# microsoft/T-MAC

Measured on AMD Instinct MI355X. Metric: W2A8 GEMV GB/s (llama-2-7B all-layer decode, N=1), higher is better.
Workload: dtype int8

## Files before the change

include/tmac_hip.h:

```cpp
#ifndef TMAC_HIP_H_
#define TMAC_HIP_H_

#include <stddef.h>
#include <stdint.h>

#ifdef __cplusplus
extern "C" {
#endif
#pragma GCC visibility push(default)

#define TMAC_HIP_OK 0
#define TMAC_HIP_E_NOMATCH (-1)
#define TMAC_HIP_E_NODEVICE (-2)
#define TMAC_HIP_E_RUNTIME (-3)
#define TMAC_HIP_E_ARG (-4)

typedef enum { TMAC_F32 = 0, TMAC_F16 = 1 } tmac_dtype_t;

#define TMAC_HIP_ABI_VERSION 1

typedef struct tmac_kcfg {
    int bm;
    int simd_n_in;
    int simd_n_out;
    int kfactor;
    int group_size;
    int lut_scales_size;
    int scales_size;
    int n_tile_num;
    int act_group_size;
    int zero_point;
    int m_groups;
} tmac_kcfg;

typedef struct tmac_hip_weights tmac_hip_weights;
typedef struct tmac_hip_workspace tmac_hip_workspace;

int32_t tmac_hip_init(int device);
const char* tmac_hip_last_error(void);
const char* tmac_hip_version(void);
int32_t tmac_hip_device_count(void);
int32_t tmac_hip_pointer_on_device(const void* p);

int32_t tmac_hip_load_kcfg(const char* path);
int32_t tmac_hip_load_kcfg_ex(const char* path, int replace);
int32_t tmac_hip_clear_kcfg(void);
int32_t tmac_hip_reset_state(void);
int32_t tmac_hip_get_kcfg(int M, int K, int N, int bits, tmac_kcfg* out);
int32_t tmac_hip_set_kcfg(int M, int K, int N, int bits, const tmac_kcfg* cfg);



int32_t tmac_hip_register_weights(tmac_hip_weights** out, const void* A_ref, const void* scales_ref,
                                  int Mw, int K, int bits, const tmac_kcfg* cfg,
                                  tmac_dtype_t host_float, tmac_dtype_t dev_float, void* stream);
int32_t tmac_hip_register_weights_dev(tmac_hip_weights** out, const void* A_ref_dev, const void* scales_ref_dev,
                                      int Mw, int K, int bits, const tmac_kcfg* cfg,
                                      tmac_dtype_t host_float, tmac_dtype_t dev_float, void* stream);
int32_t tmac_hip_free_weights(tmac_hip_weights* w);
size_t tmac_hip_weights_bytes(const tmac_hip_weights* w);

int32_t tmac_hip_workspace_create(tmac_hip_workspace** out, int maxK, int maxN);
int32_t tmac_hip_workspace_free(tmac_hip_workspace* ws);

int32_t tmac_hip_preprocessor_dev(tmac_hip_workspace* ws, const void* B_dev, tmac_dtype_t act_dtype,
                                  int K, int N, int act_group_size, void* stream);

int32_t tmac_hip_qgemm_dev(const tmac_hip_weights* w, const tmac_hip_workspace* ws, void* C_dev,
                           tmac_dtype_t out_dtype, int N, void* stream);

int32_t tmac_hip_qgemm_fused_dev(const tmac_hip_weights* const* weights, int nmat, const void* B_dev,
                                 tmac_dtype_t act_dtype, void* const* C_dev, tmac_dtype_t out_dtype, int N,
                                 void* stream);

int32_t tmac_hip_defer(int on);
int32_t tmac_hip_flush(void* stream);
int32_t tmac_hip_defer_stats(uint64_t* flushes, uint64_t* cache_hits, uint64_t* stream_launches, uint64_t* single_calls);

typedef struct tmac_hip_chain tmac_hip_chain;
int32_t tmac_hip_chain_begin(void);
int32_t tmac_hip_chain_end(tmac_hip_chain** out);
int32_t tmac_hip_chain_abort(void);
int32_t tmac_hip_chain_launch(tmac_hip_chain* chain, void* stream);
int32_t tmac_hip_chain_status(tmac_hip_chain* chain, uint32_t* error_word);
int32_t tmac_hip_chain_info(const tmac_hip_chain* chain, int op, int32_t* nops, int32_t* wpq, int32_t* grid, size_t* bytes);
int32_t tmac_hip_chain_free(tmac_hip_chain* chain);
#define TMAC_XF_NONE 0
#define TMAC_XF_NORM 1
#define TMAC_XF_GLU 2
#define TMAC_XF_GLU_NORM 4
#define TMAC_XF_GATE_SILU  0x000
#define TMAC_XF_GATE_RELU2 0x100
#define TMAC_XF_GATE_GELU  0x200
#define TMAC_XF_CARRY ((const float*)1)
typedef struct {
    int32_t kind;
    const void* in2;
    const float* residual;
    const float* gamma;
    float eps;
    float* residual_out;
    int32_t keep;
} tmac_hip_xform;
int32_t tmac_hip_chain_xform(const tmac_hip_xform* xf);
int32_t tmac_hip_qgemm_fused_xf_dev(const tmac_hip_weights* const* weights, int nmat, const void* B_dev, tmac_dtype_t act_dtype,
                                    const tmac_hip_xform* xf, void* const* C_dev, tmac_dtype_t out_dtype, void* stream);
int32_t tmac_hip_qgemm_fused_xf_rows_dev(const tmac_hip_weights* const* weights, int nmat, const void* B_dev, tmac_dtype_t act_dtype,
                                         const tmac_hip_xform* xf, void* const* C_dev, tmac_dtype_t out_dtype, int N, void* stream);
int32_t tmac_hip_debug_xf_rows_plan(const tmac_hip_weights* const* weights, int nmat, void* const* C_dev, int N, int32_t* route, int32_t* lut);
int32_t tmac_hip_debug_fused_plan(const tmac_hip_weights* const* weights, int nmat, void* const* C_dev, int N, int32_t* route, int32_t* lut);
int32_t tmac_hip_debug_route_stats(uint64_t counts[8]);
int32_t tmac_hip_debug_xf_rows(const void* B_dev, tmac_dtype_t act_dtype, const tmac_hip_xform* xf, int K, int N, float* x_out_dev,
                               void* stream);
#define TMAC_HIP_CHAIN_BLOB_BYTES 128
int32_t tmac_hip_chain_record_gather(const void* send_dev, void* recv_dev, size_t bytes_per_rank, int rank, int world);
int32_t tmac_hip_chain_export(const tmac_hip_chain* chain, void* blob_out);
int32_t tmac_hip_chain_connect(tmac_hip_chain* chain, const void* blobs_of_all_ranks, int world);
int32_t tmac_hip_chain_threads(void);
int32_t tmac_hip_chain_is_stream(const tmac_hip_chain* chain);
int32_t tmac_hip_chain_set_stamps(tmac_hip_chain* chain, unsigned long long* dev_buffer);
int32_t tmac_hip_chain_set_tap(tmac_hip_chain* chain, int32_t* dev_buffer);
int32_t tmac_hip_chain_tap_layout(const tmac_hip_chain* chain, int op, size_t* offset_ints, size_t* count_ints);
int32_t tmac_hip_debug_chain_config(int force_waves_per_quad, unsigned spin_limit);
int32_t tmac_hip_debug_chain_grid(int workgroups);
int32_t tmac_hip_debug_stream_schedule(const double* items, int n, int grid, int ncls, int target, int lpt, int32_t* out_lo, int32_t* out_w, double* out_load);

#define TMAC_HIP_COMM_ID_BYTES 128
typedef struct tmac_hip_comm tmac_hip_comm;
int32_t tmac_hip_comm_unique_id(void* id_out);
int32_t tmac_hip_comm_init(tmac_hip_comm** out, const void* id, int rank, int world);
int32_t tmac_hip_comm_allgather(tmac_hip_comm* comm, const void* send_dev, void* recv_dev, size_t bytes_per_rank, void* stream);
int32_t tmac_hip_comm_destroy(tmac_hip_comm* comm);
#define TMAC_HIP_COMM_BLOB_BYTES 128
int32_t tmac_hip_comm_init_ipc(tmac_hip_comm** out, size_t max_bytes_per_rank, int rank, int world);
int32_t tmac_hip_comm_export(const tmac_hip_comm* comm, void* blob_out);
int32_t tmac_hip_comm_connect(tmac_hip_comm* comm, const void* blobs_of_all_ranks, int world);
int32_t tmac_hip_comm_status(tmac_hip_comm* comm, uint32_t* error_word);
const char* tmac_hip_comm_last_error(void);

int32_t tmac_hip_workspace_ptrs(tmac_hip_workspace* ws, void** qlut_dev, size_t* nbytes_qlut_per_row,
                                void** lut_scales, void** lut_biases);

int32_t tmac_hip_workspace_read(tmac_hip_workspace* ws, int8_t* qlut_host, float* lut_scales_host,
                                float* lut_biases_host, int K, int N, int act_group_size, void* stream);
int32_t tmac_hip_workspace_write(tmac_hip_workspace* ws, const int8_t* qlut_host, const float* lut_scales_host,
                                 const float* lut_biases_host, int K, int N, int act_group_size, void* stream);
int32_t tmac_hip_qgemm_partial_sums(const tmac_hip_weights* w, const tmac_hip_workspace* ws,
                                    int32_t* PS_host, int N, void* stream);
int32_t tmac_hip_qgemm_fused_partial_sums(const tmac_hip_weights* w, const void* B_dev, tmac_dtype_t act_dtype,
                                          int32_t* PS_host, float* C_host, float* lut_host, int N, void* stream);
int32_t tmac_hip_selftest(const uint32_t* in_host, uint32_t* out_host, int n);
int32_t tmac_hip_selftest_mfma(const uint32_t* in_host, int32_t* out_host);
int32_t tmac_hip_set_variant(int variant);
int32_t tmac_hip_set_gemm_min_n(int n);
int32_t tmac_hip_set_fast_aggregation(int mode);
int32_t tmac_hip_debug_stream_read(const void* dev_src, size_t bytes, void* dev_sink, void* stream);
int32_t tmac_hip_debug_quad_config(int force_threads, int force_waves_per_quad);
int32_t tmac_hip_debug_stamps(unsigned long long* dev_buffer);
int32_t tmac_hip_debug_pairs_min_n(int n);
int32_t tmac_hip_debug_gemm_kernel(int which);
int32_t tmac_hip_debug_gemm_stamps(unsigned long long* dev_buffer);
int32_t tmac_hip_debug_gemm_comb_sums(const tmac_hip_weights* w, const tmac_hip_workspace* ws, int32_t* comb_host, int N, void* stream);
int32_t tmac_hip_debug_gemm_image_read(const tmac_hip_workspace* ws, int8_t* half_tables_host, float* lut_scales_host,
                                       float* lut_biases_host, float* entry_sums_host, int N, void* stream);
int32_t tmac_hip_debug_rows_kernel(int mode);
int32_t tmac_hip_debug_rows_stats(uint64_t* launches);
int32_t tmac_hip_debug_rows_plan(int K, int m_groups, int N, int32_t* r_fit, int32_t* ngroups, int32_t* cap, int32_t* live, size_t* lds_bytes);
int32_t tmac_hip_debug_rows_comb_sums(const tmac_hip_weights* w, const tmac_hip_workspace* ws, int32_t* comb_host, int N, void* stream);
int32_t tmac_hip_debug_host_runs(int on);
int32_t tmac_hip_debug_ws_fill_sync(int on);
int32_t tmac_hip_debug_defer_fail(int nth);
int32_t tmac_hip_autotune_fused(const tmac_hip_weights* const* weights, int nmat, tmac_dtype_t act_dtype,
                                tmac_dtype_t out_dtype, int* best_ft, int* best_wpq, float* best_us, float* heuristic_us);
int32_t tmac_hip_tune_save(const char* path);
int32_t tmac_hip_tune_load(const char* path);
int32_t tmac_hip_tune_clear(void);

int32_t qgemm_lut_int8(int m, int k, int n, int b, void* A, void* LUT, void* Scales, void* LUT_Scales,
                       void* LUT_Biases, void* C);
int32_t preprocessor_int8(int m, int k, int n, int b, void* B, void* LUT_Scales, void* LUT_Biases, void* QLUT);
int32_t tmac_hip_cache_clear(void);

#define TMAC_DECL_Q(bm, k, n, b) \
    int32_t qgemm_lut_t1_int8_m##bm##_k##k##_n##n##_b##b(void* A, void* LUT, void* Scales, void* LUT_Scales, void* LUT_Biases, void* C);
#define TMAC_DECL_P(m, k, n, b) \
    int32_t preprocessor_t1_int8_m##m##_k##k##_n##n##_b##b(void* B, void* LUT_Scales, void* LUT_Biases, void* QLUT);
TMAC_DECL_Q(128, 4096, 1, 2) TMAC_DECL_Q(128, 11008, 1, 2)
TMAC_DECL_P(8192, 4096, 1, 2) TMAC_DECL_P(22016, 4096, 1, 2) TMAC_DECL_P(8192, 11008, 1, 2)
TMAC_DECL_Q(1024, 4096, 1, 4) TMAC_DECL_Q(256, 4096, 1, 4) TMAC_DECL_Q(256, 11008, 1, 4)
TMAC_DECL_P(16384, 4096, 1, 4) TMAC_DECL_P(44032, 4096, 1, 4) TMAC_DECL_P(16384, 11008, 1, 4)
TMAC_DECL_Q(256, 4096, 1, 2) TMAC_DECL_Q(512, 4096, 1, 2) TMAC_DECL_Q(128, 14336, 1, 2)
TMAC_DECL_P(28672, 4096, 1, 2) TMAC_DECL_P(8192, 14336, 1, 2) TMAC_DECL_P(2048, 4096, 1, 2)
TMAC_DECL_Q(128, 8640, 1, 2) TMAC_DECL_Q(128, 3200, 1, 2) TMAC_DECL_Q(320, 3200, 1, 2)
TMAC_DECL_P(6400, 8640, 1, 2) TMAC_DECL_P(17280, 3200, 1, 2) TMAC_DECL_P(6400, 3200, 1, 2)
#undef TMAC_DECL_Q
#undef TMAC_DECL_P

#pragma GCC visibility pop
#ifdef __cplusplus
}
#endif
#endif
```

tmac_amd/binding.py:

```python
from __future__ import annotations

import ctypes as C
import os
import subprocess

HERE = os.path.dirname(os.path.abspath(__file__))
F32, F16 = 0, 1
XF_NONE, XF_NORM, XF_GLU, XF_GLU_NORM = 0, 1, 2, 4
XF_GATE_SILU, XF_GATE_RELU2, XF_GATE_GELU = 0x000, 0x100, 0x200


class TMACHipError(RuntimeError):
    def __init__(self, code: int, msg: str):
        super().__init__(f"tmac_hip error {code}: {msg}")
        self.code = code


class XForm(C.Structure):
    _fields_ = [("kind", C.c_int32), ("in2", C.c_void_p), ("residual", C.c_void_p), ("gamma", C.c_void_p), ("eps", C.c_float),
                ("residual_out", C.c_void_p), ("keep", C.c_int32)]


class KCfg(C.Structure):
    _fields_ = [(n, C.c_int) for n in ("bm", "simd_n_in", "simd_n_out", "kfactor", "group_size", "lut_scales_size",
                                       "scales_size", "n_tile_num", "act_group_size", "zero_point", "m_groups")]

    @classmethod
    def make(cls, Mw, K, bits, bm, kfactor=16, group_size=128, act_group_size=64, zero_point=True, m_groups=-1, N=1):
        per = 2 if zero_point else 1
        scales_size = m_groups if m_groups >= 1 else Mw * (K // group_size) * per
        return cls(bm, 16, 8, kfactor, group_size, N * K // act_group_size, scales_size, Mw * bits // bm,
                   act_group_size, int(bool(zero_point)) if m_groups < 1 else 0, m_groups)


def lib_path() -> str:
    return os.environ.get("TMAC_HIP_LIB") or os.path.join(HERE, "lib", "libtmac_hip.so")


def build_library(force: bool = False) -> str:
    if force:
        subprocess.run(["make", "-C", os.path.join(HERE, "csrc"), "clean"], check=True)
    subprocess.run(["make", "-s", "-j4", "-C", os.path.join(HERE, "csrc")], check=True)
    return lib_path()


_lib = None


def load_library() -> C.CDLL:
    global _lib
    if _lib is not None:
        return _lib
    p = lib_path()
    if not os.path.exists(p):
        raise ImportError(f"{p} is missing: build it with `python -c 'import __graft_entry__ as g; g.build()'` "
                          "(hipcc --offload-arch=gfx950); tmac_amd has no fallback path")
    L = C.CDLL(p)
    vp, i32, sz = C.c_void_p, C.c_int32, C.c_size_t
    sigs = {
        "tmac_hip_init": ([C.c_int], i32),
        "tmac_hip_last_error": ([], C.c_char_p),
        "tmac_hip_version": ([], C.c_char_p),
        "tmac_hip_device_count": ([], i32),
        "tmac_hip_pointer_on_device": ([vp], i32),
        "tmac_hip_load_kcfg": ([C.c_char_p], i32),
        "tmac_hip_load_kcfg_ex": ([C.c_char_p, C.c_int], i32),
        "tmac_hip_clear_kcfg": ([], i32),
        "tmac_hip_reset_state": ([], i32),
        "tmac_hip_debug_ws_fill_sync": ([C.c_int], i32),
        "tmac_hip_debug_host_runs": ([C.c_int], i32),
        "tmac_hip_get_kcfg": ([C.c_int] * 4 + [C.POINTER(KCfg)], i32),
        "tmac_hip_set_kcfg": ([C.c_int] * 4 + [C.POINTER(KCfg)], i32),
        "tmac_hip_register_weights": ([C.POINTER(vp), vp, vp, C.c_int, C.c_int, C.c_int, C.POINTER(KCfg), C.c_int, C.c_int, vp], i32),
        "tmac_hip_register_weights_dev": ([C.POINTER(vp), vp, vp, C.c_int, C.c_int, C.c_int, C.POINTER(KCfg), C.c_int, C.c_int, vp], i32),
        "tmac_hip_free_weights": ([vp], i32),
        "tmac_hip_weights_bytes": ([vp], sz),
        "tmac_hip_workspace_create": ([C.POINTER(vp), C.c_int, C.c_int], i32),
        "tmac_hip_workspace_free": ([vp], i32),
        "tmac_hip_preprocessor_dev": ([vp, vp, C.c_int, C.c_int, C.c_int, C.c_int, vp], i32),
        "tmac_hip_qgemm_dev": ([vp, vp, vp, C.c_int, C.c_int, vp], i32),
        "tmac_hip_qgemm_fused_dev": ([C.POINTER(vp), C.c_int, vp, C.c_int, C.POINTER(vp), C.c_int, C.c_int, vp], i32),
        "tmac_hip_qgemm_fused_xf_dev": ([C.POINTER(vp), C.c_int, vp, C.c_int, C.POINTER(XForm), C.POINTER(vp), C.c_int, vp], i32),
        "tmac_hip_qgemm_fused_xf_rows_dev": ([C.POINTER(vp), C.c_int, vp, C.c_int, C.POINTER(XForm), C.POINTER(vp), C.c_int, C.c_int, vp], i32),
        "tmac_hip_debug_xf_rows_plan": ([C.POINTER(vp), C.c_int, C.POINTER(vp), C.c_int, C.POINTER(C.c_int32), C.POINTER(C.c_int32)], i32),
        "tmac_hip_debug_fused_plan": ([C.POINTER(vp), C.c_int, C.POINTER(vp), C.c_int, C.POINTER(C.c_int32), C.POINTER(C.c_int32)], i32),
        "tmac_hip_debug_route_stats": ([C.POINTER(C.c_uint64)], i32),
        "tmac_hip_debug_xf_rows": ([vp, C.c_int, C.POINTER(XForm), C.c_int, C.c_int, vp, vp], i32),
        "tmac_hip_qgemm_fused_partial_sums": ([vp, vp, C.c_int, vp, vp, vp, C.c_int, vp], i32),
        "tmac_hip_workspace_ptrs": ([vp, C.POINTER(vp), C.POINTER(sz), C.POINTER(vp), C.POINTER(vp)], i32),
        "tmac_hip_workspace_read": ([vp, vp, vp, vp, C.c_int, C.c_int, C.c_int, vp], i32),
        "tmac_hip_workspace_write": ([vp, vp, vp, vp, C.c_int, C.c_int, C.c_int, vp], i32),
        "tmac_hip_qgemm_partial_sums": ([vp, vp, vp, C.c_int, vp], i32),
        "tmac_hip_debug_gemm_kernel": ([C.c_int], i32),
        "tmac_hip_debug_gemm_stamps": ([vp], i32),
        "tmac_hip_debug_gemm_comb_sums": ([vp, vp, vp, C.c_int, vp], i32),
        "tmac_hip_debug_rows_kernel": ([C.c_int], i32),
        "tmac_hip_debug_rows_stats": ([C.POINTER(C.c_uint64)], i32),
        "tmac_hip_debug_rows_plan": ([C.c_int, C.c_int, C.c_int, C.POINTER(C.c_int32), C.POINTER(C.c_int32), C.POINTER(C.c_int32), C.POINTER(C.c_int32), C.POINTER(C.c_size_t)], i32),
        "tmac_hip_debug_rows_comb_sums": ([vp, vp, vp, C.c_int, vp], i32),
        "tmac_hip_debug_gemm_image_read": ([vp, vp, vp, vp, vp, C.c_int, vp], i32),
        "tmac_hip_set_variant": ([C.c_int], i32),
        "tmac_hip_set_gemm_min_n": ([C.c_int], i32),
        "tmac_hip_set_fast_aggregation": ([C.c_int], i32),
        "tmac_hip_debug_stream_read": ([vp, sz, vp, vp], i32),
        "tmac_hip_autotune_fused": ([C.c_void_p, C.c_int, C.c_int, C.c_int, C.POINTER(C.c_int), C.POINTER(C.c_int),
                                     C.POINTER(C.c_float), C.POINTER(C.c_float)], i32),
        "tmac_hip_tune_save": ([C.c_char_p], i32),
        "tmac_hip_tune_load": ([C.c_char_p], i32),
        "tmac_hip_tune_clear": ([], i32),
        "tmac_hip_comm_unique_id": ([vp], i32),
        "tmac_hip_comm_init": ([C.POINTER(vp), vp, C.c_int, C.c_int], i32),
        "tmac_hip_comm_allgather": ([vp, vp, vp, sz, vp], i32),
        "tmac_hip_comm_destroy": ([vp], i32),
        "tmac_hip_comm_init_ipc": ([C.POINTER(vp), sz, C.c_int, C.c_int], i32),
        "tmac_hip_comm_export": ([vp, vp], i32),
        "tmac_hip_comm_connect": ([vp, vp, C.c_int], i32),
        "tmac_hip_comm_status": ([vp, C.POINTER(C.c_uint32)], i32),
        "tmac_hip_comm_last_error": ([], C.c_char_p),
        "tmac_hip_defer": ([C.c_int], i32),
        "tmac_hip_flush": ([vp], i32),
        "tmac_hip_debug_defer_fail": ([C.c_int], i32),
        "tmac_hip_defer_stats": ([C.POINTER(C.c_uint64)] * 4, i32),
        "tmac_hip_chain_begin": ([], i32),
        "tmac_hip_chain_end": ([C.POINTER(vp)], i32),
        "tmac_hip_chain_launch": ([vp, vp], i32),
        "tmac_hip_chain_status": ([vp, C.POINTER(C.c_uint32)], i32),
        "tmac_hip_chain_info": ([vp, C.c_int, C.POINTER(i32), C.POINTER(i32), C.POINTER(i32), C.POINTER(sz)], i32),
        "tmac_hip_chain_xform": ([C.POINTER(XForm)], i32),
        "tmac_hip_chain_free": ([vp], i32),
        "tmac_hip_chain_set_stamps": ([vp, vp], i32),
        "tmac_hip_chain_set_tap": ([vp, vp], i32),
        "tmac_hip_chain_tap_layout": ([vp, C.c_int, C.POINTER(sz), C.POINTER(sz)], i32),
        "tmac_hip_chain_threads": ([], i32),
        "tmac_hip_chain_is_stream": ([vp], i32),
        "tmac_hip_chain_record_gather": ([vp, vp, sz, C.c_int, C.c_int], i32),
        "tmac_hip_chain_export": ([vp, vp], i32),
        "tmac_hip_chain_connect": ([vp, vp, C.c_int], i32),
        "tmac_hip_debug_chain_grid": ([C.c_int], i32),
        "tmac_hip_debug_stream_schedule": ([C.POINTER(C.c_double), C.c_int, C.c_int, C.c_int, C.c_int, C.c_int, C.POINTER(C.c_int32), C.POINTER(C.c_int32), C.POINTER(C.c_double)], i32),
        "tmac_hip_debug_chain_config": ([C.c_int, C.c_uint], i32),
        "tmac_hip_debug_quad_config": ([C.c_int, C.c_int], i32),
        "tmac_hip_selftest": ([vp, vp, C.c_int], i32),
        "tmac_hip_selftest_mfma": ([vp, vp], i32),
        "tmac_hip_cache_clear": ([], i32),
        "qgemm_lut_int8": ([C.c_int] * 4 + [vp] * 6, i32),
        "preprocessor_int8": ([C.c_int] * 4 + [vp] * 4, i32),
    }
    optional = {"tmac_hip_chain_is_stream", "tmac_hip_chain_xform", "tmac_hip_qgemm_fused_xf_dev", "tmac_hip_qgemm_fused_xf_rows_dev", "tmac_hip_debug_xf_rows", "tmac_hip_debug_xf_rows_plan", "tmac_hip_debug_fused_plan", "tmac_hip_debug_route_stats", "tmac_hip_comm_init_ipc", "tmac_hip_comm_export", "tmac_hip_comm_connect", "tmac_hip_comm_status",
                "tmac_hip_debug_rows_kernel", "tmac_hip_debug_rows_stats", "tmac_hip_debug_rows_plan", "tmac_hip_debug_rows_comb_sums"} if os.environ.get("TMAC_HIP_LIB") else set()
    for name, (argt, rest) in sigs.items():
        try:
            fn = getattr(L, name)
        except AttributeError:
            if name in optional:
                continue
            raise
        fn.argtypes, fn.restype = argt, rest
    _lib = L
    return L


def lib() -> C.CDLL:
    return load_library()


def check(rc: int) -> None:
    if rc != 0:
        raise TMACHipError(rc, load_library().tmac_hip_last_error().decode())


def check_count(rc: int) -> int:
    if rc < 0:
        raise TMACHipError(rc, load_library().tmac_hip_last_error().decode())
    return rc
```

tmac_amd/csrc/tmac_chain.h:

```cpp
#pragma once
#include <hip/hip_runtime.h>
#include <stdint.h>

namespace tmac {

#ifndef TMAC_CHAIN_FT
#define TMAC_CHAIN_FT 768
#endif
constexpr int CHAIN_FT = TMAC_CHAIN_FT;
constexpr int CHAIN_NWV = CHAIN_FT / 64;
constexpr int CHAIN_RED = 4;
constexpr int CHAIN_US_FLOATS = 48;
constexpr int CHAIN_US_MAX_GROUPS = 8;

struct ChainMat {
    const uint4* W;
    const void* SC;
    void* C;
    uint4* GR;
    int Mw;
    int q_end;
};

struct ChainOp {
    ChainMat m[4];
    int q_end[4];
    const void* in;
    int in_gran;
    int nmat;
    int K, nu, nst, tstride, G, GP, nsg, gs_shift;
    int wpq, ipi;
    int wpq_inv;
    int total_q;
    int q_per, q_extra;
    int m_groups;
    int ipi_inv;
    const void* in2;
    const float* res;
    const float* gamma;
    float* res_out;
    int xf_kind;
    int xf_flags;
    int eps_bits;
    int epi;
    const void* img;
    int img_u4;
    int wg_lo;
};
static_assert(sizeof(ChainOp) == 320, "ChainOp is copied to LDS in 16-byte pieces");

struct ChainArgs {
    const ChainOp* ops;
    int nops;
    unsigned* ctl;
    int out_f16;
    unsigned spin_limit;
    int buf_u4;
    int poll_sleep;
    int poll_delay;
    int issue_first;
    int poll_mode;
    int poll_grid;
    unsigned long long arena_base;
    unsigned long long arena_half;
    unsigned long long peer_base[7];
    int npeer;
    int xforms;
    int carry_floats;
    int tmp_floats, gam_floats;
    int ext_floats;
    int32_t* tap;
    const unsigned long long* tap_off;
    unsigned long long* stamps;
    int gates;
};

hipError_t launch_decode_chain_b1(const ChainArgs& a, bool zp, bool sc_f16, int sm, int grid, size_t lds_bytes, hipStream_t st, int* resident);
hipError_t launch_decode_chain_b2(const ChainArgs& a, bool zp, bool sc_f16, int sm, int grid, size_t lds_bytes, hipStream_t st, int* resident);
hipError_t launch_decode_chain_b3(const ChainArgs& a, bool zp, bool sc_f16, int sm, int grid, size_t lds_bytes, hipStream_t st, int* resident);
hipError_t launch_decode_chain_b4(const ChainArgs& a, bool zp, bool sc_f16, int sm, int grid, size_t lds_bytes, hipStream_t st, int* resident);
hipError_t launch_decode_chain_g2_b1(const ChainArgs& a, bool zp, bool sc_f16, int sm, int grid, size_t lds_bytes, hipStream_t st, int* resident);
hipError_t launch_decode_chain_g2_b2(const ChainArgs& a, bool zp, bool sc_f16, int sm, int grid, size_t lds_bytes, hipStream_t st, int* resident);
hipError_t launch_decode_chain_g2_b3(const ChainArgs& a, bool zp, bool sc_f16, int sm, int grid, size_t lds_bytes, hipStream_t st, int* resident);
hipError_t launch_decode_chain_g2_b4(const ChainArgs& a, bool zp, bool sc_f16, int sm, int grid, size_t lds_bytes, hipStream_t st, int* resident);
inline hipError_t launch_decode_chain(const ChainArgs& a, int bits, bool zp, bool sc_f16, int sm, bool g2, int grid, size_t lds_bytes, hipStream_t st,
                                      int* resident = nullptr) {
    if (g2) {
        switch (bits) {
            case 1: return launch_decode_chain_g2_b1(a, zp, sc_f16, sm, grid, lds_bytes, st, resident);
            case 2: return launch_decode_chain_g2_b2(a, zp, sc_f16, sm, grid, lds_bytes, st, resident);
            case 3: return launch_decode_chain_g2_b3(a, zp, sc_f16, sm, grid, lds_bytes, st, resident);
            case 4: return launch_decode_chain_g2_b4(a, zp, sc_f16, sm, grid, lds_bytes, st, resident);
            default: return hipErrorInvalidValue;
        }
    }
    switch (bits) {
        case 1: return launch_decode_chain_b1(a, zp, sc_f16, sm, grid, lds_bytes, st, resident);
        case 2: return launch_decode_chain_b2(a, zp, sc_f16, sm, grid, lds_bytes, st, resident);
        case 3: return launch_decode_chain_b3(a, zp, sc_f16, sm, grid, lds_bytes, st, resident);
        case 4: return launch_decode_chain_b4(a, zp, sc_f16, sm, grid, lds_bytes, st, resident);
        default: return hipErrorInvalidValue;
    }
}
inline int chain_buf_u4(int K) {
    const int nu = K / 32, nst = (nu + 63) / 64;
    return 4 * 65 * nst + (2 * nst * 32 * 4 + 15) / 16 + CHAIN_US_FLOATS / 4;
}
inline int chain_xf_region_floats(int K) {
    const int P = K / 8, nr = (P + CHAIN_FT - 1) / CHAIN_FT, PS = ((P < CHAIN_FT ? P : CHAIN_FT) + 63) & ~63;
    return nr * 2 * PS * 4;
}
inline size_t chain_lds_bytes(int buf_u4, int nops, int xf_floats = 0) {
    return (size_t)2 * buf_u4 * 16 + sizeof(float) * 2 * CHAIN_NWV * 4 * CHAIN_RED + sizeof(ChainOp) * (size_t)nops + sizeof(float) * (32 + (size_t)xf_floats);
}

#ifndef TMAC_CHAIN_STAMPS
#define TMAC_CHAIN_STAMPS 0
#endif

#ifndef TMAC_STREAM_NLW
#define TMAC_STREAM_NLW 12
#endif
constexpr int STREAM_NLW = TMAC_STREAM_NLW;
constexpr int STREAM_FT = (STREAM_NLW + 1) * 64;
struct StreamArgs {
    const ChainOp* ops;
    int nops;
    int out_f16;
    int buf_u4;
    int nsplit;
    int ncls;
    int vmax;
    const int* nvis;
    const int* roles;
    int32_t* tap;
    const unsigned long long* tap_off;
    unsigned long long* stamps;
};
enum { SR_NST = 0, SR_IPI, SR_NSG, SR_GSH, SR_NU, SR_QE0, SR_QE1, SR_QE2, SR_QPER, SR_QEXTRA, SR_IT_LO, SR_IT_HI, SR_TSTRIDE, SR_OP , SR_WPQ,
       SR_WLO , SR_COMMON };
enum { SRW_NQ = 0 , SRW_NSTEPS, SRW_H, SRW_QS, SRW_INTS };
constexpr int STREAM_ROLE_INTS = SR_COMMON + SRW_INTS * STREAM_NLW;
inline int stream_img_u4(int K) { return (chain_buf_u4(K) + 63) & ~63; }
inline size_t stream_lds_bytes(int buf_u4, int nops, bool qw = false) {
    size_t b = (size_t)2 * buf_u4 * 16 + sizeof(float) * 2 * STREAM_NLW * (qw ? 16 : 4) * CHAIN_RED + sizeof(ChainOp) * (size_t)nops;
#ifdef TMAC_STREAM_STAMPS
    b += 32 * (STREAM_NLW + 1);
#endif
    return b;
}
hipError_t launch_lut_images(const ChainOp* d_ops, int nops, int max_nst, int sm, bool sc_f16, hipStream_t st);
hipError_t launch_gemv_stream(const StreamArgs& a, int bits, bool zp, bool sc_f16, int sm, bool qw, bool g2, int grid, size_t lds_bytes, hipStream_t st);

}
```

tmac_amd/csrc/tmac_chain_host.cpp:

```cpp
#include "tmac_chain_host.h"
#include <algorithm>
#include <array>
#include <memory>
#include <optional>

using namespace tmac_host;

static thread_local std::vector<ChainRecOp>* g_chain_rec = nullptr;
static thread_local std::vector<ChainRecGather>* g_chain_gat = nullptr;
static thread_local std::optional<XfSpec> g_chain_xf;
bool tmac_host::chain_recording() { return g_chain_rec != nullptr; }
void tmac_host::chain_clear_xform() { g_chain_xf.reset(); }

int32_t tmac_host::chain_record(const tmac_hip_weights* const* wl, int nmat, const void* B_dev, tmac_dtype_t act_dtype,
                            void* const* C_list, tmac_dtype_t out_dtype, int N) {
    if (N != 1) { chain_clear_xform(); return fail(TMAC_HIP_E_NOMATCH, "a decode chain records N = 1 calls only"); }
    ChainRecOp op;
    for (int i = 0; i < nmat; ++i) {
        if (!wl[i] || !C_list[i]) { chain_clear_xform(); return fail(TMAC_HIP_E_ARG, "null matrix or output"); }
        op.w.push_back(wl[i]);
        op.C.push_back(C_list[i]);
    }
    op.B = B_dev; op.act = act_dtype; op.out = out_dtype;
    op.xf = g_chain_xf.value_or(XfSpec{});
    chain_clear_xform();
    g_chain_rec->push_back(op);
    return TMAC_HIP_OK;
}

extern "C" int32_t tmac_hip_chain_xform(const tmac_hip_xform* xf) {
    if (!g_chain_rec) return fail(TMAC_HIP_E_ARG, "no chain is being recorded on this thread");
    if (!xf) return fail(TMAC_HIP_E_ARG, "null transform");
    XfSpec spec;
    const int32_t rc = xf_resolve(xf, XF_SITE_CHAIN, &spec);
    if (rc) return rc;
    g_chain_xf = spec;
    return TMAC_HIP_OK;
}

extern "C" int32_t tmac_hip_chain_begin(void) {
    if (g_chain_rec) return fail(TMAC_HIP_E_ARG, "a chain is already being recorded on this thread");
    g_chain_rec = new std::vector<ChainRecOp>();
    g_chain_gat = new std::vector<ChainRecGather>();
    chain_clear_xform();
    return TMAC_HIP_OK;
}

extern "C" int32_t tmac_hip_chain_abort(void) {
    if (!g_chain_rec) return TMAC_HIP_OK;
    delete g_chain_rec;
    delete g_chain_gat;
    g_chain_rec = nullptr;
    g_chain_gat = nullptr;
    chain_clear_xform();
    return TMAC_HIP_OK;
}

extern "C" int32_t tmac_hip_chain_end(tmac_hip_chain** out) {
    if (!g_chain_rec) return fail(TMAC_HIP_E_ARG, "no chain is being recorded on this thread");
    std::vector<ChainRecOp> rec;
    std::vector<ChainRecGather> gat;
    rec.swap(*g_chain_rec);
    gat.swap(*g_chain_gat);
    delete g_chain_rec;
    delete g_chain_gat;
    g_chain_rec = nullptr;
    g_chain_gat = nullptr;
    if (!out) return fail(TMAC_HIP_E_ARG, "null argument");
    return chain_build(rec, gat, out);
}

extern "C" int32_t tmac_hip_chain_record_gather(const void* send_dev, void* recv_dev, size_t bytes_per_rank, int rank, int world) {
    if (!g_chain_rec) return fail(TMAC_HIP_E_ARG, "no chain is being recorded on this thread");
    if (!send_dev || !recv_dev || !bytes_per_rank || world < 1 || world > 8 || rank < 0 || rank >= world)
        return fail(TMAC_HIP_E_ARG, "bad gather (1..8 ranks)");
    g_chain_gat->push_back(ChainRecGather{send_dev, recv_dev, bytes_per_rank, rank, world, g_chain_rec->size()});
    return TMAC_HIP_OK;
}
bool tmac_host::chain_record_gather_if_recording(const void* send_dev, void* recv_dev, size_t bytes_per_rank, int rank, int world, int32_t* rc) {
    if (!g_chain_rec) return false;
    *rc = tmac_hip_chain_record_gather(send_dev, recv_dev, bytes_per_rank, rank, world);
    return true;
}

static int chain_pick_wpq(int total_q, int nst, int grid, int nwv = CHAIN_NWV) {
    int best = 1;
    long best_cost = 1L << 60;
    for (int wpq = 1; wpq <= 4; ++wpq) {
        if (nwv % wpq || (wpq > 1 && wpq > nst)) continue;
        const long ipi = nwv / wpq;
        const long cnt = (total_q + grid - 1) / grid;
        const long iters = (cnt + ipi - 1) / ipi;
        const long steps = (nst + wpq - 1) / wpq;
        if (iters * steps < best_cost) { best_cost = iters * steps; best = wpq; }
    }
    return best;
}

extern "C" int32_t tmac_hip_chain_free(tmac_hip_chain* c) {
    if (!c) return TMAC_HIP_OK;
    const int32_t brc = defer_barrier();
    for (void* p : c->peers) if (p) (void)hipIpcCloseMemHandle(p);
    if (c->arena) (void)hipFree(c->arena);
    if (c->images) (void)hipFree(c->images);
    if (c->d_tap_off) (void)hipFree(c->d_tap_off);
    if (c->d_ops) (void)hipFree(c->d_ops);
    if (c->ctl) (void)hipFree(c->ctl);
    delete c;
    return brc;
}

static void set_wpq(ChainOp& o, int wpq, int nwv) {
    o.wpq = wpq;
    o.ipi = nwv / wpq;
    o.wpq_inv = (65536 + wpq - 1) / wpq;
    o.ipi_inv = (65536 + o.ipi - 1) / o.ipi;
}

static int cls_lo(int cl, int grid, int ncls) { return (cl * grid + ncls - 1) / ncls; }
static void stream_schedule(const std::vector<double>& items, int grid, int ncls, int target, bool lpt, std::vector<int>& blk_lo, std::vector<int>& blk_w,
                            std::vector<std::vector<int>>& visits) {
    const int nop = (int)items.size();
    const double visit_fixed = 8.0;
    blk_lo.assign(nop, 0); blk_w.assign(nop, ncls);
    visits.assign(ncls, std::vector<int>());
    double best_span = 0;
    int best_cap = 0;
    for (int pass = 0; pass < 2; ++pass) {
        for (int cap = ncls; cap >= 1; cap >>= 1) {
            if (pass == 1 && cap != best_cap) continue;
            std::vector<double> load(ncls, 0.0);
            std::vector<std::vector<int>> vis(ncls);
            std::vector<int> order(nop), wof(nop);
            for (int i = 0; i < nop; ++i) {
                int n = 1;
                while (n < cap && items[i] * n / grid < target) n <<= 1;
                order[i] = i; wof[i] = ncls / n;
            }
            if (lpt)
                std::stable_sort(order.begin(), order.end(), [&](int x, int y) {
                    if (wof[x] != wof[y]) return wof[x] > wof[y];
                    return items[x] > items[y];
                });
            for (int oi = 0; oi < nop; ++oi) {
                const int i = order[oi], w = wof[i];
                int bb = 0;
                double bl = 1e300;
                for (int b0 = 0; b0 + w <= ncls; b0 += w) {
                    double m = 0;
                    for (int k = b0; k < b0 + w; ++k) m = load[k] > m ? load[k] : m;
                    if (m < bl) { bl = m; bb = b0; }
                }
                const int wg = cls_lo(bb + w, grid, ncls) - cls_lo(bb, grid, ncls);
                for (int k = bb; k < bb + w; ++k) { load[k] += visit_fixed + items[i] / wg; vis[k].push_back(i); }
                if (pass == 1) { blk_lo[i] = bb; blk_w[i] = w; }
            }
            double span = 0;
            for (int k = 0; k < ncls; ++k) span = load[k] > span ? load[k] : span;
            if (pass == 0 && (best_cap == 0 || span < best_span * 0.999)) { best_span = span; best_cap = cap; }
            if (pass == 1) visits.swap(vis);
        }
    }
}
extern "C" int32_t tmac_hip_debug_stream_schedule(const double* items, int n, int grid, int ncls, int target, int lpt, int32_t* out_lo, int32_t* out_w, double* out_load) {
    if (!items || n < 1 || grid < 1 || ncls < 1 || ncls > 16 || (ncls & (ncls - 1)) || ncls > grid || !out_lo || !out_w) return fail(TMAC_HIP_E_ARG, "bad schedule query");
    std::vector<double> it(items, items + n);
    std::vector<int> lo, w;
    std::vector<std::vector<int>> vis;
    stream_schedule(it, grid, ncls, target, lpt != 0, lo, w, vis);
    for (int i = 0; i < n; ++i) { out_lo[i] = lo[i]; out_w[i] = w[i]; }
    if (out_load)
        for (int k = 0; k < ncls; ++k) {
            out_load[k] = 0;
            for (int i : vis[k]) {
                const int wg = cls_lo(lo[i] + w[i], grid, ncls) - cls_lo(lo[i], grid, ncls);
                out_load[k] += it[i] / wg;
            }
        }
    return TMAC_HIP_OK;
}

static int env_int(const char* name, int dflt) {
    const char* e = getenv(name);
    return e ? atoi(e) : dflt;
}
struct BuildKnobs {
    int wpq = g_knobs.chain_wpq;
    bool glu_epilogue = env_int("TMAC_CHAIN_GLU_EPILOGUE", 1) != 0;
    bool stream = env_int("TMAC_CHAIN_STREAM", 1) != 0;
    int ncls = env_int("TMAC_STREAM_NCLS", 16);
    int visit_items = env_int("TMAC_STREAM_VISIT_ITEMS", 160);
    int qw = env_int("TMAC_STREAM_QW", -1);
    bool lpt = env_int("TMAC_STREAM_LPT", 1) != 0;
    int split = env_int("TMAC_STREAM_SPLIT", 2);
    int split_bits = env_int("TMAC_STREAM_SPLIT_BITS", 3);
    bool split_bits_set = getenv("TMAC_STREAM_SPLIT_BITS") != nullptr;
    int poll_sleep = env_int("TMAC_CHAIN_POLL_SLEEP", 8), poll_delay = env_int("TMAC_CHAIN_POLL_DELAY", 4);
    int issue_first = env_int("TMAC_CHAIN_ISSUE_FIRST", -1), poll_mode = env_int("TMAC_CHAIN_POLL_MODE", 0), poll_grid = env_int("TMAC_CHAIN_POLL_GRID", 0);
    explicit BuildKnobs(int grid) {
        ncls = std::min(std::max(ncls, 1), 16);
        while (ncls > grid || (ncls & (ncls - 1))) --ncls;
    }
};

struct Src { int op, mat; };
struct ChainFlow {
    std::vector<Range> in_r;
    std::vector<std::vector<Range>> out_r;
    std::vector<Src> src, src2;
    std::vector<std::vector<char>> consumed, gathered;
    std::vector<std::vector<char>> dep;
    std::vector<char> epi_of, glu_in_producer;
};
static Src latest_output(const std::vector<ChainRecOp>& rec, const ChainFlow& f, size_t i, const Range& r, const void* p, bool* partial) {
    *partial = false;
    for (size_t j = i; j-- > 0;)
        for (size_t m = 0; m < rec[j].C.size(); ++m)
            if (overlap(r, f.out_r[j][m])) { *partial = rec[j].C[m] != p; return Src{(int)j, (int)m}; }
    return Src{-1, -1};
}
static int32_t analyse_flow(const std::vector<ChainRecOp>& rec, const std::vector<ChainRecGather>& gat, tmac_dtype_t out, ChainFlow& f) {
    const size_t n = rec.size(), out_esz = out == TMAC_F16 ? 2 : 4;
    f.in_r.resize(n); f.out_r.resize(n);
    for (size_t i = 0; i < n; ++i) {
        f.in_r[i] = act_range(rec[i]);
        for (size_t m = 0; m < rec[i].w.size(); ++m) f.out_r[i].push_back(out_range(rec[i], m, out));
        for (size_t m = 0; m < f.out_r[i].size(); ++m)
            for (size_t m2 = 0; m2 < m; ++m2)
                if (overlap(f.out_r[i][m], f.out_r[i][m2])) return fail(TMAC_HIP_E_ARG, "op %zu: outputs %zu and %zu overlap", i, m2, m);
    }
    f.src.assign(n, Src{-1, -1}); f.src2.assign(n, Src{-1, -1});
    f.consumed.resize(n); f.gathered.resize(n);
    for (size_t i = 0; i < n; ++i) { f.consumed[i].assign(rec[i].w.size(), 0); f.gathered[i].assign(rec[i].w.size(), 0); }
    bool partial;
    for (size_t i = 0; i < n; ++i) {
        const ChainRecGather* via = nullptr;
        for (const ChainRecGather& g : gat)
            if (g.pos <= i && g.recv == rec[i].B && (!via || g.pos >= via->pos)) via = &g;
        if (via) {
            for (size_t j = via->pos; j-- > 0 && f.src[i].op < 0;)
                for (size_t m = 0; m < rec[j].C.size(); ++m)
                    if (rec[j].C[m] == via->send) {
                        if (via->bytes != (size_t)rec[j].w[m]->s.Mw * out_esz)
                            return fail(TMAC_HIP_E_ARG, "op %zu: the exchange step gathers %zu bytes per rank, output %zu of op %zu has %zu", i, via->bytes, m, j,
                                        (size_t)rec[j].w[m]->s.Mw * out_esz);
                        if ((size_t)rec[i].w[0]->s.K > (size_t)via->world * rec[j].w[m]->s.Mw)
                            return fail(TMAC_HIP_E_ARG, "op %zu reads %d activations from a gather of %d x %d rows", i, rec[i].w[0]->s.K, via->world, rec[j].w[m]->s.Mw);
                        f.src[i] = Src{(int)j, (int)m};
                        f.consumed[j][m] = 1; f.gathered[j][m] = 1;
                        break;
                    }
            if (f.src[i].op < 0) return fail(TMAC_HIP_E_ARG, "op %zu reads a gathered buffer whose send side no earlier call of the chain writes", i);
            continue;
        }
        const Src s = latest_output(rec, f, i, f.in_r[i], rec[i].B, &partial);
        if (partial)
            return fail(TMAC_HIP_E_NOMATCH, "op %zu reads activations that overlap output %zu of op %zu without being that output: "
                                            "not representable as a hand-off", i, (size_t)s.mat, (size_t)s.op);
        if (s.op >= 0) { f.src[i] = s; f.consumed[s.op][s.mat] = 1; }
    }
    for (size_t i = 0; i < n; ++i) {
        if (!xf_has_glu(rec[i].xf)) continue;
        const Range r2{(const char*)rec[i].xf.in2, (const char*)rec[i].xf.in2 + (size_t)rec[i].w[0]->s.K * 2};
        const Src s = latest_output(rec, f, i, r2, rec[i].xf.in2, &partial);
        if (partial) return fail(TMAC_HIP_E_NOMATCH, "op %zu: the GLU's second vector overlaps output %zu of op %zu without being that output", i, (size_t)s.mat, (size_t)s.op);
        if (s.op >= 0) {
            if (f.gathered[s.op][s.mat]) return fail(TMAC_HIP_E_NOMATCH, "op %zu: a gathered output as the second vector of a GLU is not covered", i);
            f.src2[i] = s; f.consumed[s.op][s.mat] = 1;
        }
        if ((f.src2[i].op >= 0) != (f.src[i].op >= 0))
            return fail(TMAC_HIP_E_NOMATCH, "op %zu: the two vectors of a GLU must both be outputs of the chain or both be external", i);
    }
    f.dep.assign(n, std::vector<char>(n, 0));
    for (size_t k = 0; k < n; ++k) {
        if (f.src[k].op >= 0) {
            f.dep[k] = f.dep[f.src[k].op];
            f.dep[k][f.src[k].op] = 1;
        }
        if (f.src2[k].op >= 0) {
            for (size_t q = 0; q < n; ++q) f.dep[k][q] |= f.dep[f.src2[k].op][q];
            f.dep[k][f.src2[k].op] = 1;
        }
    }
    return TMAC_HIP_OK;
}

static char chain_epi(const XfSpec& s) { return (char)(1 + s.gate); }
static void fill_chain_xf(ChainOp& o, const XfSpec& s, bool in_producer) {
    const bool norm = s.kind == TMAC_XF_NORM, glu_norm = s.kind == TMAC_XF_GLU_NORM;
    o.xf_kind = glu_norm ? TMAC_XF_NORM : (s.kind == TMAC_XF_GLU && in_producer) ? TMAC_XF_NONE : s.kind;
    if (o.xf_kind == TMAC_XF_GLU) o.xf_flags |= s.gate << 8;
    if (norm) {
        o.xf_flags |= (s.carry ? 2 : 0) | (s.keep ? 4 : 0);
        o.res = s.residual; o.res_out = s.residual_out;
    }
    if (norm || glu_norm) { o.gamma = s.gamma; memcpy(&o.eps_bits, &s.eps, 4); }
}

static void plan_glu_epilogue(const std::vector<ChainRecOp>& rec, ChainFlow& f, int grid, const BuildKnobs& kn) {
    const size_t n = rec.size();
    f.epi_of.assign(n, 0); f.glu_in_producer.assign(n, 0);
    if (!kn.glu_epilogue) return;
    std::vector<std::vector<int>> readers(n);
    for (size_t j = 0; j < n; ++j) readers[j].assign(rec[j].w.size(), 0);
    for (size_t i = 0; i < n; ++i) {
        if (f.src[i].op >= 0) ++readers[f.src[i].op][f.src[i].mat];
        if (f.src2[i].op >= 0) ++readers[f.src2[i].op][f.src2[i].mat];
    }
    for (size_t i = 0; i < n; ++i) {
        if (!xf_has_glu(rec[i].xf) || f.src[i].op < 0 || f.src2[i].op != f.src[i].op || f.src[i].mat != 0 || f.src2[i].mat != 1) continue;
        const size_t j = (size_t)f.src[i].op;
        if (rec[j].w.size() != 2 || rec[j].w[0]->s.Mw != rec[j].w[1]->s.Mw || f.gathered[j][0] || f.gathered[j][1] || readers[j][0] != 1 || f.epi_of[j]) continue;
        const Shape& sj = rec[j].w[0]->s;
        const int nqj = 2 * sj.nquads(), nstj = (sj.K / 32 + 63) / 64;
        const int wq = kn.wpq ? kn.wpq : chain_pick_wpq(nqj, nstj, grid);
        if (CHAIN_NWV % wq || ((CHAIN_NWV / wq) & 1)) continue;
        f.epi_of[j] = chain_epi(rec[i].xf); f.glu_in_producer[i] = 1;
        if (readers[j][1] == 1) f.consumed[j][1] = 0;
    }
}

constexpr size_t NO_IMAGE = ~(size_t)0;
struct ChainLayout {
    std::vector<std::array<size_t, 4>> gr;
    std::vector<size_t> in, in2;
    int maxK = 0;
};

static int32_t describe_ops(const std::vector<ChainRecOp>& rec, const ChainFlow& f, const BuildKnobs& kn, tmac_hip_chain& c, ChainLayout& lay) {
    const size_t n = rec.size();
    c.ops.resize(n);
    lay.gr.assign(n, {NO_IMAGE, NO_IMAGE, NO_IMAGE, NO_IMAGE});
    lay.in.assign(n, 0); lay.in2.assign(n, 0);
    for (size_t i = 0; i < n; ++i) {
        const ChainRecOp& r = rec[i];
        ChainOp& o = c.ops[i];
        memset(&o, 0, sizeof(o));
        const Shape& s0 = r.w[0]->s;
        const Src src = f.src[i], src2 = f.src2[i];
        if (r.act != TMAC_F16 && r.act != TMAC_F32) return fail(TMAC_HIP_E_NOMATCH, "op %zu: the decode chain takes fp16 or fp32 activations", i);
        if (r.act == TMAC_F32 && (src.op >= 0 || xf_has_glu(r.xf)))
            return fail(TMAC_HIP_E_NOMATCH, "op %zu: fp32 activations are covered for vectors in memory (an earlier output is handed over as fp16), without a GLU transform", i);
        if ((r.out == TMAC_F16) != (c.out_f16 != 0)) return fail(TMAC_HIP_E_NOMATCH, "op %zu: one output dtype per chain", i);
        if (s0.K > 8 * 3 * CHAIN_FT) return fail(TMAC_HIP_E_NOMATCH, "op %zu: K = %d beyond the decode chain's %d", i, s0.K, 8 * 3 * CHAIN_FT);
        if (((s0.m_groups >= 1) ? 2 : 0) != c.sm) return fail(TMAC_HIP_E_NOMATCH, "op %zu: per-group and unified scales cannot share a chain", i);
        int gu = 1;
        if (c.sm == 2) {
            if (s0.ags != s0.K || s0.K % 64 || s0.m_groups > CHAIN_US_MAX_GROUPS)
                return fail(TMAC_HIP_E_NOMATCH, "op %zu: the unified-scale chain covers one act group per row (act_group_size == K) and up to %d scales per matrix",
                            i, CHAIN_US_MAX_GROUPS);
        } else {
            gu = s0.gs / 32;
            if (s0.ags != 64 || s0.gs < 64 || (gu & (gu - 1)) || s0.K % s0.gs || s0.K % 64)
                return fail(TMAC_HIP_E_NOMATCH, "op %zu: the decode chain covers per-group scales (group >= 64, power of two) with act groups of 64", i);
            if (s0.gs == 64) c.g2 = 1;
        }
        int nq = 0;
        for (size_t m = 0; m < r.w.size(); ++m) {
            const tmac_hip_weights* w = r.w[m];
            const Shape& a = w->s;
            if (layout_of(a) != L_QUAD || !w->tiled_ok || w->fa) return fail(TMAC_HIP_E_NOMATCH, "op %zu matrix %zu is not registered in the QUAD layout", i, m);
            if (a.K != s0.K || a.bits != c.bits || a.gs != s0.gs || a.ags != s0.ags || a.zero_point != c.zp || a.m_groups != s0.m_groups ||
                (w->sc_dtype == F16) != (c.sc_f16 != 0))
                return fail(TMAC_HIP_E_ARG, "op %zu: the matrices of a chain share bits, zero points and scale dtype; those of an op also K and group size", i);
            if (c.sm == 2 && a.Mw % a.m_groups) return fail(TMAC_HIP_E_NOMATCH, "op %zu matrix %zu: rows not divisible by m_groups", i, m);
            nq += a.nquads();
            o.m[m].W = (const uint4*)w->W; o.m[m].SC = w->SC; o.m[m].C = r.C[m]; o.m[m].Mw = a.Mw; o.m[m].q_end = nq;
            if (f.consumed[i][m]) {
                if (r.out != TMAC_F16) return fail(TMAC_HIP_E_NOMATCH, "op %zu: outputs consumed inside the chain must be fp16", i);
                if (f.gathered[i][m] && a.Mw % 4) return fail(TMAC_HIP_E_NOMATCH, "op %zu: row shards of a gathered output must be whole row quads", i);
                const size_t nq_img = (size_t)a.nquads() * (f.gathered[i][m] ? c.world : 1);
                const size_t my_off = f.gathered[i][m] ? (size_t)c.rank * a.nquads() * 16 : 0;
                lay.gr[i][m] = c.arena_bytes + my_off;
                c.layout_hash = (c.layout_hash ^ (nq_img * 16 + i * 4 + m)) * 1099511628211ull;
                c.arena_bytes += (nq_img * 16 + 255) & ~(size_t)255;
            }
            c.bytes += w->w_bytes + w->sc_bytes;
        }
        o.nmat = (int)r.w.size();
        for (int m = 0; m < 4; ++m) o.q_end[m] = (m < o.nmat - 1) ? o.m[m].q_end : 0x7fffffff;
        o.K = s0.K; o.nu = s0.K / 32; o.nst = (o.nu + 63) / 64; o.tstride = o.nst * 64 + 1;
        o.G = s0.K / 64; o.GP = o.nst * 32; o.nsg = c.sm == 2 ? 1 : s0.K / s0.gs;
        o.gs_shift = 0;
        for (int g = gu; g > 1; g >>= 1) ++o.gs_shift;
        o.m_groups = c.sm == 2 ? s0.m_groups : 0;
        o.total_q = nq;
        const int wpq = kn.wpq ? kn.wpq : chain_pick_wpq(nq, o.nst, c.grid);
        if (CHAIN_NWV % wpq) return fail(TMAC_HIP_E_ARG, "waves per quad must divide %d", CHAIN_NWV);
        set_wpq(o, wpq, CHAIN_NWV);
        if (nq / c.grid + 1 + o.ipi >= 4096) return fail(TMAC_HIP_E_NOMATCH, "op %zu: too many rows per workgroup for the decode chain", i);
        o.q_per = nq / c.grid; o.q_extra = nq % c.grid;
        if (f.epi_of[i]) { o.epi = f.epi_of[i]; c.xforms = 1; if (o.epi > 1) c.gates = 1; o.q_per = (nq / 2) / c.grid; o.q_extra = (nq / 2) % c.grid; }
        if (src.op >= 0) {
            const ChainMat& pm = c.ops[src.op].m[src.mat];
            const bool via_gather = f.gathered[src.op][src.mat] != 0;
            if (!via_gather && pm.Mw != o.K) return fail(TMAC_HIP_E_ARG, "op %zu reads an output of %d rows as %d activations", i, pm.Mw, o.K);
            const size_t my_off = via_gather ? (size_t)c.rank * ((pm.Mw + 3) / 4) * 16 : 0;
            lay.in[i] = lay.gr[src.op][src.mat] - my_off; o.in_gran = 1;
        } else {
            o.in = r.B; o.in_gran = 0;
            if (r.act == TMAC_F32) { o.in_gran = 2; c.xforms = 1;
                if (chain_xf_region_floats(s0.K) > c.ext_floats) c.ext_floats = chain_xf_region_floats(s0.K); }
        }
        if (r.xf.kind != TMAC_XF_NONE) {
            const XfSpec& xf = r.xf;
            const int rf = chain_xf_region_floats(o.K);
            const bool reads_glu = xf.kind == TMAC_XF_GLU && !f.glu_in_producer[i];
            const bool runs = xf.kind != TMAC_XF_GLU || reads_glu;
            if (xf.kind == TMAC_XF_GLU_NORM && !f.glu_in_producer[i])
                return fail(TMAC_HIP_E_NOMATCH, "op %zu: a GLU_NORM transform is recorded only where the call in front publishes silu(in) * in2 itself (in and in2 "
                                                "outputs 0 and 1 of one earlier two-matrix call that nothing else reads through a hand-off, not gathered, "
                                                "TMAC_CHAIN_GLU_EPILOGUE != 0, an even number of row quads per workgroup iteration): launch these calls one by one", i);
            if (runs) {
                c.xforms = 1;
                if (o.K > 2 * 8 * CHAIN_FT)
                    return fail(TMAC_HIP_E_NOMATCH, "op %zu: a %s transform is covered up to K = %d%s", i, xf.kind == TMAC_XF_NORM ? "NORM" : xf.kind == TMAC_XF_GLU ? "GLU" : "GLU_NORM",
                                2 * 8 * CHAIN_FT, xf.kind == TMAC_XF_GLU_NORM ? " (the NORM's limit)" : "");
            }
            if (xf.kind == TMAC_XF_NORM) {
                if (o.K > 8192 && (xf.keep || xf.carry)) return fail(TMAC_HIP_E_NOMATCH, "op %zu: a kept residual vector is covered up to K = 8192", i);
                if (xf.carry && c.carry_K != o.K) return fail(TMAC_HIP_E_ARG, "op %zu: no earlier NORM of the chain keeps a vector of %d values", i, o.K);
                if (xf.keep) { c.carry_K = o.K; if (rf > c.carry_floats) c.carry_floats = rf; }
            }
            if (runs && !xf.keep && rf > c.tmp_floats) c.tmp_floats = rf;
            if (xf.gamma && rf > c.gam_floats) c.gam_floats = rf;
            if (reads_glu) {
                if (xf.gate) c.gates = 1;
                if (src2.op >= 0) {
                    const ChainMat& p2 = c.ops[src2.op].m[src2.mat];
                    if (p2.Mw != o.K) return fail(TMAC_HIP_E_ARG, "op %zu: the GLU's second vector has %d rows, K = %d", i, p2.Mw, o.K);
                    lay.in2[i] = lay.gr[src2.op][src2.mat];
                } else o.in2 = xf.in2;
            }
            fill_chain_xf(o, xf, f.glu_in_producer[i] != 0);
        }
        o.in_gran |= 1 << 8;
        if (o.K > lay.maxK) lay.maxK = o.K;
    }
    return TMAC_HIP_OK;
}

static int32_t check_hazards(const std::vector<ChainRecOp>& rec, const ChainFlow& f, const std::vector<ChainOp>& ops) {
    const size_t n = rec.size();
    auto all_past = [&](size_t i, size_t k) {
        for (size_t j = i; j < k; ++j)
            if (f.dep[k][j] && ops[j].q_per >= 1) return true;
        return false;
    };
    for (size_t k = 0; k < n; ++k)
        for (size_t m = 0; m < f.out_r[k].size(); ++m)
            for (size_t i = 0; i < k; ++i) {
                if (f.src[i].op < 0 && overlap(f.out_r[k][m], f.in_r[i]) && !all_past(i, k))
                    return fail(TMAC_HIP_E_NOMATCH, "op %zu overwrites activations that op %zu reads from memory and nothing in the chain orders the two "
                                                    "(no hand-off path from an op in which every workgroup owns rows): launch these calls one by one", k, i);
                for (size_t m2 = 0; m2 < f.out_r[i].size(); ++m2)
                    if (overlap(f.out_r[k][m], f.out_r[i][m2]) && !f.dep[k][i])
                        return fail(TMAC_HIP_E_NOMATCH, "ops %zu and %zu write overlapping outputs and nothing in the chain orders them", i, k);
            }
    std::vector<std::vector<Range>> xf_rd(n);
    std::vector<Range> xf_wr(n, Range{nullptr, nullptr});
    for (size_t i = 0; i < n; ++i) {
        const XfSpec& xf = rec[i].xf;
        const size_t K = (size_t)rec[i].w[0]->s.K;
        if (xf.residual) xf_rd[i].push_back(Range{(const char*)xf.residual, (const char*)xf.residual + K * 4});
        if (xf.in2 && f.src2[i].op < 0) xf_rd[i].push_back(Range{(const char*)xf.in2, (const char*)xf.in2 + K * 2});
        if (xf.gamma) xf_rd[i].push_back(Range{(const char*)xf.gamma, (const char*)xf.gamma + K * 4});
        if (xf.residual_out) xf_wr[i] = Range{(const char*)xf.residual_out, (const char*)xf.residual_out + K * 4};
    }
    for (size_t k = 0; k < n; ++k) {
        for (size_t i = 0; i < n; ++i)
            for (const Range& r : xf_rd[i]) {
                for (size_t m = 0; m < f.out_r[k].size(); ++m)
                    if (overlap(f.out_r[k][m], r) && (i >= k || !all_past(i, k)))
                        return fail(TMAC_HIP_E_NOMATCH, "op %zu writes output %zu over a vector that the transform of op %zu reads from memory and nothing in the "
                                                        "chain orders the writer behind every reader", k, m, i);
                if (xf_wr[k].lo && overlap(xf_wr[k], r) && (i >= k || !all_past(i, k)))
                    return fail(TMAC_HIP_E_NOMATCH, "op %zu: residual_out overlaps a vector that the transform of op %zu reads from memory (a later NORM of the "
                                                    "launch takes the kept vector, TMAC_XF_CARRY)", k, i);
            }
        if (!xf_wr[k].lo) continue;
        for (size_t i = 0; i < n; ++i) {
            if (f.src[i].op < 0 && overlap(xf_wr[k], f.in_r[i]) && (i >= k || !all_past(i, k)))
                return fail(TMAC_HIP_E_NOMATCH, "op %zu: residual_out overlaps activations that op %zu reads from memory", k, i);
            for (size_t m = 0; m < f.out_r[i].size(); ++m)
                if (overlap(xf_wr[k], f.out_r[i][m])) return fail(TMAC_HIP_E_NOMATCH, "op %zu: residual_out overlaps output %zu of op %zu", k, m, i);
            if (i != k && xf_wr[i].lo && overlap(xf_wr[k], xf_wr[i])) return fail(TMAC_HIP_E_NOMATCH, "ops %zu and %zu: overlapping residual_out vectors", i, k);
        }
    }
    return TMAC_HIP_OK;
}

static bool independent(const std::vector<ChainRecOp>& rec, const std::vector<ChainRecGather>& gat, const ChainFlow& f, const std::vector<ChainOp>& ops) {
    if (!gat.empty()) return false;
    for (size_t i = 0; i < rec.size(); ++i)
        if (f.src[i].op >= 0 || f.src2[i].op >= 0 || rec[i].xf.kind != TMAC_XF_NONE || ops[i].epi) return false;
    return true;
}
struct StreamPlan {
    std::vector<ChainOp> ops;
    std::vector<size_t> img_off;
    std::vector<int32_t> roles;
    size_t img_bytes = 0, lds_bytes = 0;
    int buf_u4 = 0, max_nst = 0, ncls = 1, vmax = 1, nsplit = 1;
    bool qw = true;
};
static std::optional<StreamPlan> plan_stream(std::vector<ChainOp> ops, int bits, bool g2, int grid, const BuildKnobs& kn) {
    StreamPlan p;
    p.ops = std::move(ops);
    const int nop = (int)p.ops.size(), ncls = p.ncls = kn.ncls;
    p.img_off.resize(nop);
    for (int i = 0; i < nop; ++i) {
        ChainOp& o = p.ops[i];
        o.img_u4 = stream_img_u4(o.K);
        p.img_off[i] = p.img_bytes;
        p.img_bytes += (size_t)o.img_u4 * 16;
        if (o.img_u4 > p.buf_u4) p.buf_u4 = o.img_u4;
        if (o.nst > p.max_nst) p.max_nst = o.nst;
        o.in_gran &= 2;
    }
    const int nwv = STREAM_NLW;
    {
        double it64 = 0, it16 = 0;
        for (const ChainOp& o : p.ops) {
            for (int m = 0; m < o.nmat; ++m) if (((o.m[m].Mw + 3) / 4) % 4) p.qw = false;
            it64 += (double)o.total_q * o.nst; it16 += (double)(o.total_q / 4) * ((o.nu + 15) / 16);
        }
        if (kn.qw == 0 || (kn.qw < 0 && bits >= 3 && it16 > 0.85 * it64)) p.qw = false;
    }
    const bool qw = p.qw;
    auto op_q = [&](const ChainOp& o) { return qw ? o.total_q / 4 : o.total_q; };
    auto op_nst = [&](const ChainOp& o) { return qw ? (o.nu + 15) / 16 : o.nst; };
    std::vector<int> blk_lo, blk_w;
    std::vector<std::vector<int>> visits;
    {
        std::vector<double> items(nop);
        for (int i = 0; i < nop; ++i) items[i] = (double)op_q(p.ops[i]) * op_nst(p.ops[i]);
        stream_schedule(items, grid, ncls, kn.visit_items, kn.lpt, blk_lo, blk_w, visits);
    }
    for (int i = 0; i < nop; ++i) {
        ChainOp& o = p.ops[i];
        const int wlo = cls_lo(blk_lo[i], grid, ncls), wcnt = cls_lo(blk_lo[i] + blk_w[i], grid, ncls) - wlo;
        o.wg_lo = wlo;
        const int tq = op_q(o), nstw = op_nst(o);
        set_wpq(o, (!kn.wpq || nwv % o.wpq || o.wpq > nstw) ? chain_pick_wpq(tq, nstw, wcnt, nwv) : o.wpq, nwv);
        o.q_per = tq / wcnt; o.q_extra = tq % wcnt;
        if (tq / wcnt + 1 + o.ipi >= 4096) return std::nullopt;
        if (qw) for (int m = 0; m < 4; ++m) { if (o.q_end[m] != 0x7fffffff) o.q_end[m] /= 4; o.m[m].q_end /= 4; }
    }
    int vmax = 1;
    for (int k = 0; k < ncls; ++k) if ((int)visits[k].size() > vmax) vmax = (int)visits[k].size();
    p.vmax = vmax;
    const size_t lds2 = stream_lds_bytes(p.buf_u4, (vmax + 1) / 2, qw);
    p.lds_bytes = stream_lds_bytes(p.buf_u4, vmax, qw);
    const int split_bits = (g2 && !kn.split_bits_set && kn.split_bits > 2) ? 2 : kn.split_bits;
    if (kn.split >= 2 && bits <= split_bits && vmax >= 2 && 2 * lds2 + 2048 <= 160 * 1024) { p.nsplit = 2; p.lds_bytes = lds2; }
    for (int ns = 3; ns <= kn.split && ns <= 4; ++ns) {
        const size_t ldsn = stream_lds_bytes(p.buf_u4, (vmax + ns - 1) / ns, qw);
        if (p.nsplit == ns - 1 && vmax >= ns && ns * (ldsn + 1024) <= 160 * 1024) { p.nsplit = ns; p.lds_bytes = ldsn; }
    }
    if (p.lds_bytes > 160 * 1024) return std::nullopt;
    p.roles.assign((size_t)STREAM_ROLE_INTS * ncls * vmax + ncls, 0);
    for (int k = 0; k < ncls; ++k) {
        p.roles[(size_t)STREAM_ROLE_INTS * ncls * vmax + k] = (int32_t)visits[k].size();
        for (size_t v = 0; v < visits[k].size(); ++v) {
            const int i = visits[k][v];
            const ChainOp& o = p.ops[i];
            int32_t* r = p.roles.data() + ((size_t)k * vmax + v) * STREAM_ROLE_INTS;
            const int nstw = op_nst(o);
            r[SR_NST] = nstw; r[SR_IPI] = o.ipi; r[SR_NSG] = o.nsg; r[SR_GSH] = o.gs_shift; r[SR_NU] = o.nu;
            r[SR_QE0] = o.q_end[0]; r[SR_QE1] = o.q_end[1]; r[SR_QE2] = o.q_end[2];
            r[SR_QPER] = o.q_per; r[SR_QEXTRA] = o.q_extra;
            r[SR_IT_LO] = (o.q_per + o.ipi - 1) / o.ipi; r[SR_IT_HI] = (o.q_per + o.ipi) / o.ipi;
            r[SR_TSTRIDE] = o.tstride; r[SR_OP] = i; r[SR_WPQ] = o.wpq; r[SR_WLO] = o.wg_lo;
            for (int wl = 0; wl < STREAM_NLW; ++wl) {
                int32_t* rw = r + SR_COMMON + SRW_INTS * wl;
                const int qs = wl / o.wpq, h = wl - qs * o.wpq;
                auto nq = [&](int cnt) { return qs < cnt ? (cnt - 1 - qs) / o.ipi + 1 : 0; };
                rw[SRW_NQ] = nq(o.q_per) | (nq(o.q_per + 1) << 16);
                rw[SRW_NSTEPS] = h < nstw ? (nstw - h + o.wpq - 1) / o.wpq : 0;
                rw[SRW_H] = h; rw[SRW_QS] = qs;
            }
        }
    }
    return p;
}

static int32_t commit_stream(tmac_hip_chain& c, StreamPlan& p) {
    const size_t role_bytes = p.roles.size() * sizeof(int32_t);
    if (hipMalloc(&c.images, p.img_bytes + role_bytes) != hipSuccess || hipMemset(c.images, 0, p.img_bytes) != hipSuccess ||
        hipMemcpy(static_cast<char*>(c.images) + p.img_bytes, p.roles.data(), role_bytes, hipMemcpyHostToDevice) != hipSuccess)
        return fail(TMAC_HIP_E_RUNTIME, "LUT image allocation failed (%zu bytes)", p.img_bytes + role_bytes);
    c.roles = reinterpret_cast<const int*>(static_cast<char*>(c.images) + p.img_bytes);
    c.nvis = c.roles + (size_t)STREAM_ROLE_INTS * p.ncls * p.vmax;
    c.ncls = p.ncls; c.vmax = p.vmax; c.qw = p.qw; c.nsplit = p.nsplit; c.max_nst = p.max_nst;
    c.ops = std::move(p.ops);
    for (size_t i = 0; i < c.ops.size(); ++i) c.ops[i].img = static_cast<const char*>(c.images) + p.img_off[i];
    c.stream = true; c.buf_u4 = p.buf_u4; c.lds_bytes = p.lds_bytes; c.xforms = 0;
    return TMAC_HIP_OK;
}
static int32_t commit(tmac_hip_chain& c, const ChainLayout& lay) {
    if (!c.stream) {
        c.buf_u4 = chain_buf_u4(lay.maxK);
        c.lds_bytes = chain_lds_bytes(c.buf_u4, (int)c.ops.size(), c.carry_floats + c.tmp_floats + c.gam_floats + c.ext_floats);
        if (c.lds_bytes > 160 * 1024)
            return fail(TMAC_HIP_E_NOMATCH, "%zu calls with K up to %d need %zu bytes of LDS (LUT buffers + call descriptors): record shorter chains",
                        c.ops.size(), lay.maxK, c.lds_bytes);
        ChainArgs probe;
        memset(&probe, 0, sizeof(probe));
        probe.nops = 1;
        int resident = 0;
        hipError_t e = launch_decode_chain(probe, c.bits, c.zp != 0, c.sc_f16 != 0, c.sm, c.g2 != 0, c.grid, c.lds_bytes, nullptr, &resident);
        if (e == hipErrorInvalidValue) return fail(TMAC_HIP_E_NOMATCH, "no decode-chain kernel for this configuration");
        if (e != hipSuccess || resident < 1)
            return fail(TMAC_HIP_E_NOMATCH, "the decode chain's workgroup does not fit a compute unit (%s, %zu bytes of LDS)",
                        e == hipSuccess ? "occupancy 0" : hipGetErrorString(e), c.lds_bytes);
    }
    if (c.arena_bytes) {
        const hipError_t ea = c.world > 1 ? hipExtMallocWithFlags(&c.arena, 2 * c.arena_bytes, hipDeviceMallocFinegrained)
                                          : hipMalloc(&c.arena, 2 * c.arena_bytes);
        if (ea != hipSuccess || hipMemset(c.arena, 0, 2 * c.arena_bytes) != hipSuccess)
            return fail(TMAC_HIP_E_RUNTIME, "hand-off arena allocation failed (%zu bytes)", 2 * c.arena_bytes);
        char* const base = static_cast<char*>(c.arena);
        for (size_t i = 0; i < c.ops.size(); ++i) {
            ChainOp& o = c.ops[i];
            for (int m = 0; m < o.nmat; ++m)
                if (lay.gr[i][m] != NO_IMAGE) o.m[m].GR = reinterpret_cast<uint4*>(base + lay.gr[i][m]);
            if (o.in_gran & 1) o.in = base + lay.in[i];
            if ((o.in_gran & 1) && o.xf_kind == TMAC_XF_GLU) o.in2 = base + lay.in2[i];
        }
    }
    c.connected = c.world == 1;
    if (hipMalloc((void**)&c.d_ops, sizeof(ChainOp) * c.ops.size()) != hipSuccess ||
        hipMemcpy(c.d_ops, c.ops.data(), sizeof(ChainOp) * c.ops.size(), hipMemcpyHostToDevice) != hipSuccess)
        return fail(TMAC_HIP_E_RUNTIME, "descriptor upload failed");
    const unsigned ctl0[4] = {1u, 0u, 0u, 0u};
    if (hipMalloc((void**)&c.ctl, sizeof(ctl0)) != hipSuccess || hipMemcpy(c.ctl, ctl0, sizeof(ctl0), hipMemcpyHostToDevice) != hipSuccess)
        return fail(TMAC_HIP_E_RUNTIME, "control word allocation failed");
    if (hipStreamSynchronize(nullptr) != hipSuccess) return fail(TMAC_HIP_E_RUNTIME, "hand-off buffer initialisation failed");
    return TMAC_HIP_OK;
}

struct ChainFree { void operator()(tmac_hip_chain* c) const { (void)tmac_hip_chain_free(c); } };

int32_t tmac_host::chain_build(const std::vector<ChainRecOp>& rec, const std::vector<ChainRecGather>& gat, tmac_hip_chain** out) {
    *out = nullptr;
    if (rec.empty()) return fail(TMAC_HIP_E_ARG, "nothing was recorded");
    int32_t rc = ensure_device();
    if (rc) return rc;
    int dev = 0, cus = 0;
    HIP_TRY(hipGetDevice(&dev));
    HIP_TRY(hipDeviceGetAttribute(&cus, hipDeviceAttributeMultiprocessorCount, dev));
    if (cus < 1) return fail(TMAC_HIP_E_RUNTIME, "no compute units reported");
    std::unique_ptr<tmac_hip_chain, ChainFree> c(new tmac_hip_chain());
    c->grid = (g_knobs.chain_grid > 0 && g_knobs.chain_grid < cus) ? g_knobs.chain_grid : cus;
    const BuildKnobs kn(c->grid);
    for (const ChainRecGather& g : gat) {
        if (g.world != gat[0].world || g.rank != gat[0].rank) return fail(TMAC_HIP_E_ARG, "the exchange steps of a chain share rank and world size");
        c->rank = g.rank; c->world = g.world;
    }
    const tmac_hip_weights* w0 = rec[0].w[0];
    c->bits = w0->s.bits; c->zp = w0->s.zero_point; c->sc_f16 = w0->sc_dtype == F16; c->out_f16 = rec[0].out == TMAC_F16;
    c->sm = (w0->s.m_groups >= 1) ? 2 : 0;
    if (c->bits < 1 || c->bits > 4) return fail(TMAC_HIP_E_NOMATCH, "the decode chain is built for 1- to 4-bit weights");

    ChainFlow flow;
    if ((rc = analyse_flow(rec, gat, rec[0].out, flow)) != TMAC_HIP_OK) return rc;
    plan_glu_epilogue(rec, flow, c->grid, kn);
    ChainLayout lay;
    if ((rc = describe_ops(rec, flow, kn, *c, lay)) != TMAC_HIP_OK) return rc;
    if ((rc = check_hazards(rec, flow, c->ops)) != TMAC_HIP_OK) return rc;
    std::optional<StreamPlan> plan;
    if (kn.stream && independent(rec, gat, flow, c->ops)) plan = plan_stream(c->ops, c->bits, c->g2 != 0, c->grid, kn);
    if (plan && (rc = commit_stream(*c, *plan)) != TMAC_HIP_OK) return rc;
    if ((rc = commit(*c, lay)) != TMAC_HIP_OK) return rc;
    c->poll_sleep = kn.poll_sleep; c->poll_delay = kn.poll_delay; c->issue_first = kn.issue_first; c->poll_mode = kn.poll_mode; c->poll_grid = kn.poll_grid;
    *out = c.release();
    return TMAC_HIP_OK;
}

extern "C" int32_t tmac_hip_debug_chain_grid(int workgroups) {
    if (workgroups < 0) return fail(TMAC_HIP_E_ARG, "negative grid");
    g_knobs.chain_grid = workgroups;
    return TMAC_HIP_OK;
}

extern "C" int32_t tmac_hip_debug_chain_config(int force_wpq, unsigned spin_limit) {
    if (force_wpq < 0 || (force_wpq && CHAIN_NWV % force_wpq)) return fail(TMAC_HIP_E_ARG, "waves per quad must divide %d", CHAIN_NWV);
    g_knobs.chain_wpq = force_wpq;
    if (spin_limit) g_knobs.chain_spin_limit = spin_limit;
    return TMAC_HIP_OK;
}
```

tmac_amd/csrc/tmac_chain_host.h:

```cpp
#pragma once
#include "tmac_host.h"

struct tmac_hip_chain {
    std::vector<tmac::ChainOp> ops;
    tmac::ChainOp* d_ops = nullptr;
    unsigned* ctl = nullptr;
    void* arena = nullptr;
    size_t arena_bytes = 0;
    unsigned long long layout_hash = 0;
    int rank = 0, world = 1;
    std::vector<void*> peers;
    bool connected = false;
    int bits = 0, zp = 0, sc_f16 = 0, out_f16 = 0;
    int sm = 0;
    int grid = 0, buf_u4 = 0;
    size_t lds_bytes = 0;
    unsigned long long* stamps = nullptr;
    int32_t* tap = nullptr;
    unsigned long long* d_tap_off = nullptr;
    size_t bytes = 0;
    int xforms = 0, carry_floats = 0;
    int gates = 0;
    int tmp_floats = 0, gam_floats = 0, ext_floats = 0, carry_K = 0;
    int poll_sleep = 8, poll_delay = 4, issue_first = -1, poll_mode = 0, poll_grid = 0;
    hipStream_t last_stream = nullptr;
    bool launched = false;
    bool stream = false;
    void* images = nullptr;
    int max_nst = 0;
    const int* roles = nullptr;
    const int* nvis = nullptr;
    int ncls = 1, vmax = 0;
    bool qw = false;
    int nsplit = 1;
    int g2 = 0;
};

namespace tmac_host {

struct ChainRecOp {
    std::vector<const tmac_hip_weights*> w;
    const void* B;
    std::vector<void*> C;
    tmac_dtype_t act, out;
    XfSpec xf;
};
struct ChainRecGather {
    const void* send;
    const void* recv;
    size_t bytes;
    int rank, world;
    size_t pos;
};

struct Range { const char* lo; const char* hi; };
inline bool overlap(const Range& a, const Range& b) { return a.lo < b.hi && b.lo < a.hi; }
inline Range act_range(const ChainRecOp& r) { return Range{(const char*)r.B, (const char*)r.B + (size_t)r.w[0]->s.K * (r.act == TMAC_F32 ? 4 : 2)}; }
inline Range out_range(const ChainRecOp& r, size_t m, tmac_dtype_t out) {
    return Range{(const char*)r.C[m], (const char*)r.C[m] + (size_t)r.w[m]->s.Mw * (out == TMAC_F16 ? 2 : 4)};
}

int32_t chain_build(const std::vector<ChainRecOp>& rec, const std::vector<ChainRecGather>& gat, tmac_hip_chain** out);

}
```

tmac_amd/csrc/tmac_chain_launch.cpp:

```cpp
#include "tmac_chain_host.h"

using namespace tmac_host;

extern "C" int32_t tmac_hip_chain_launch(tmac_hip_chain* c, void* stream) {
    bind_thread_device();
    const int32_t brc = defer_barrier();
    if (brc) return brc;
    if (!c) return fail(TMAC_HIP_E_ARG, "null chain");
    hipStream_t st = (hipStream_t)stream;
    if (c->launched && st != c->last_stream && hipStreamQuery(c->last_stream) != hipSuccess) {
        (void)hipGetLastError();
        return fail(TMAC_HIP_E_ARG, "the chain is still in flight on another stream: synchronise it first, or record one chain per stream");
    }
    if (!c->connected) return fail(TMAC_HIP_E_ARG, "a row-sharded chain must be connected to its peers first (tmac_hip_chain_export / tmac_hip_chain_connect)");
    if (c->stream) {
        hipError_t e = launch_lut_images(c->d_ops, (int)c->ops.size(), c->max_nst, c->sm, c->sc_f16 != 0, st);
        if (e != hipSuccess) return fail(TMAC_HIP_E_RUNTIME, "LUT image launch: %s", hipGetErrorString(e));
        StreamArgs sa;
        memset(&sa, 0, sizeof(sa));
        sa.ops = c->d_ops; sa.nops = (int)c->ops.size(); sa.out_f16 = c->out_f16; sa.buf_u4 = c->buf_u4; sa.nsplit = c->nsplit; sa.roles = c->roles; sa.stamps = c->stamps;
        sa.ncls = c->ncls; sa.vmax = c->vmax; sa.nvis = c->nvis; sa.tap = c->tap; sa.tap_off = c->d_tap_off;
        e = launch_gemv_stream(sa, c->bits, c->zp != 0, c->sc_f16 != 0, c->sm, c->qw, c->g2 != 0, c->grid, c->lds_bytes, st);
        if (e != hipSuccess) return fail(TMAC_HIP_E_RUNTIME, "stream launch: %s", hipGetErrorString(e));
        c->last_stream = st; c->launched = true;
        return TMAC_HIP_OK;
    }
    ChainArgs a;
    memset(&a, 0, sizeof(a));
    a.ops = c->d_ops; a.nops = (int)c->ops.size(); a.ctl = c->ctl; a.out_f16 = c->out_f16;
    a.arena_base = reinterpret_cast<unsigned long long>(c->arena); a.arena_half = c->arena_bytes;
    a.npeer = (int)c->peers.size();
    for (int p = 0; p < a.npeer; ++p) a.peer_base[p] = reinterpret_cast<unsigned long long>(c->peers[p]);
    a.spin_limit = g_knobs.chain_spin_limit; a.buf_u4 = c->buf_u4; a.stamps = c->stamps;
    a.xforms = c->xforms; a.gates = c->gates; a.carry_floats = c->carry_floats; a.tmp_floats = c->tmp_floats; a.gam_floats = c->gam_floats; a.ext_floats = c->ext_floats;
    {
        static const int force_xf = [] { const char* e = getenv("TMAC_HIP_CHAIN_FORCE_XF"); return e && e[0] == '1' ? 1 : 0; }();
        if (force_xf) a.xforms = 1;
    }
    if (c->tap) { a.tap = c->tap; a.tap_off = c->d_tap_off; a.xforms = 1; }
    a.poll_sleep = c->poll_sleep; a.poll_delay = c->poll_delay; a.issue_first = c->issue_first; a.poll_mode = c->poll_mode; a.poll_grid = c->poll_grid;
    hipError_t e = launch_decode_chain(a, c->bits, c->zp != 0, c->sc_f16 != 0, c->sm, c->g2 != 0, c->grid, c->lds_bytes, st);
    if (e == hipErrorInvalidValue) return fail(TMAC_HIP_E_NOMATCH, "no decode-chain kernel for this configuration");
    if (e != hipSuccess) return fail(TMAC_HIP_E_RUNTIME, "decode chain launch: %s", hipGetErrorString(e));
    c->last_stream = st; c->launched = true;
    return TMAC_HIP_OK;
}

struct ChainBlob {
    hipIpcMemHandle_t handle;
    unsigned long long arena_bytes, layout_hash;
    int rank, world;
};
static_assert(sizeof(ChainBlob) <= TMAC_HIP_CHAIN_BLOB_BYTES, "blob size");

extern "C" int32_t tmac_hip_chain_export(const tmac_hip_chain* c, void* blob_out) {
    if (!c || !blob_out) return fail(TMAC_HIP_E_ARG, "null argument");
    if (!c->arena) return fail(TMAC_HIP_E_ARG, "the chain hands nothing over");
    ChainBlob b;
    memset(&b, 0, sizeof(b));
    HIP_TRY(hipIpcGetMemHandle(&b.handle, c->arena));
    b.arena_bytes = 2 * c->arena_bytes; b.layout_hash = c->layout_hash; b.rank = c->rank; b.world = c->world;
    memset(blob_out, 0, TMAC_HIP_CHAIN_BLOB_BYTES);
    memcpy(blob_out, &b, sizeof(b));
    return TMAC_HIP_OK;
}

extern "C" int32_t tmac_hip_chain_connect(tmac_hip_chain* c, const void* blobs, int world) {
    if (!c || !blobs) return fail(TMAC_HIP_E_ARG, "null argument");
    if (world != c->world) return fail(TMAC_HIP_E_ARG, "the chain was recorded for %d ranks, %d blobs given", c->world, world);
    if (c->connected && c->world > 1) return fail(TMAC_HIP_E_ARG, "the chain is already connected");
    bind_thread_device();
    for (int r = 0; r < world; ++r) {
        ChainBlob b;
        memcpy(&b, (const char*)blobs + (size_t)r * TMAC_HIP_CHAIN_BLOB_BYTES, sizeof(b));
        if (b.rank != r || b.world != world || b.arena_bytes != 2 * c->arena_bytes || b.layout_hash != c->layout_hash)
            return fail(TMAC_HIP_E_ARG, "rank %d recorded a different chain (its blob does not match this rank's hand-off layout)", r);
        if (r == c->rank) continue;
        void* p = nullptr;
        hipError_t e = hipIpcOpenMemHandle(&p, b.handle, hipIpcMemLazyEnablePeerAccess);
        if (e != hipSuccess) {
            for (void* q : c->peers) if (q) (void)hipIpcCloseMemHandle(q);
            c->peers.clear();
            return fail(TMAC_HIP_E_RUNTIME, "hipIpcOpenMemHandle of rank %d's hand-off arena: %s", r, hipGetErrorString(e));
        }
        c->peers.push_back(p);
    }
    c->connected = true;
    return TMAC_HIP_OK;
}

extern "C" int32_t tmac_hip_chain_status(tmac_hip_chain* c, uint32_t* error_word) {
    if (!c || !error_word) return fail(TMAC_HIP_E_ARG, "null argument");
    unsigned ctl[4];
    HIP_TRY(hipMemcpy(ctl, c->ctl, sizeof(ctl), hipMemcpyDeviceToHost));
    *error_word = ctl[2];
    if (ctl[2] || ctl[1]) {
        if (ctl[1] && c->world > 1)
            return fail(TMAC_HIP_E_RUNTIME, "a row-sharded chain was interrupted inside a launch (%u of its workgroups exited): the ranks' generations differ now -- "
                                            "free the chain on every rank, record and connect it again", ctl[1]);
        if (ctl[1] && c->arena) HIP_TRY(hipMemset(c->arena, 0, 2 * c->arena_bytes));
        const unsigned fresh[4] = {ctl[0], 0u, 0u, 0u};
        HIP_TRY(hipMemcpy(c->ctl, fresh, sizeof(fresh), hipMemcpyHostToDevice));
    }
    return TMAC_HIP_OK;
}

extern "C" int32_t tmac_hip_chain_info(const tmac_hip_chain* c, int op, int32_t* nops, int32_t* wpq, int32_t* grid, size_t* bytes) {
    if (!c) return fail(TMAC_HIP_E_ARG, "null chain");
    if (nops) *nops = (int32_t)c->ops.size();
    if (grid) *grid = c->grid;
    if (bytes) *bytes = c->bytes;
    if (wpq) {
        if (op < 0 || op >= (int)c->ops.size()) return fail(TMAC_HIP_E_ARG, "op index out of range");
        *wpq = c->ops[op].wpq;
    }
    return TMAC_HIP_OK;
}

static std::vector<unsigned long long> tap_offsets(const tmac_hip_chain* c) {
    std::vector<unsigned long long> off(c->ops.size() + 1, 0);
    for (size_t i = 0; i < c->ops.size(); ++i)
        off[i + 1] = off[i] + (unsigned long long)4 * c->ops[i].total_q * (c->sm == 2 ? c->bits : c->ops[i].G);
    return off;
}
extern "C" int32_t tmac_hip_chain_tap_layout(const tmac_hip_chain* c, int op, size_t* offset_ints, size_t* count_ints) {
    if (!c) return fail(TMAC_HIP_E_ARG, "null chain");
    if (op < 0 || op > (int)c->ops.size()) return fail(TMAC_HIP_E_ARG, "op index out of range");
    const std::vector<unsigned long long> off = tap_offsets(c);
    if (offset_ints) *offset_ints = (size_t)off[op];
    if (count_ints) *count_ints = op < (int)c->ops.size() ? (size_t)(off[op + 1] - off[op]) : 0;
    return TMAC_HIP_OK;
}
extern "C" int32_t tmac_hip_chain_set_tap(tmac_hip_chain* c, int32_t* dev_buffer) {
    if (!c) return fail(TMAC_HIP_E_ARG, "null chain");
    if (!dev_buffer) { c->tap = nullptr; return TMAC_HIP_OK; }
    for (const ChainOp& o : c->ops)
        if (o.epi) return fail(TMAC_HIP_E_NOMATCH, "the tap does not cover calls whose row quads are dealt in gate / up pairs (GLU in the producer)");
    bind_thread_device();
    if (!c->d_tap_off) {
        const std::vector<unsigned long long> off = tap_offsets(c);
        if (hipMalloc((void**)&c->d_tap_off, off.size() * sizeof(unsigned long long)) != hipSuccess ||
            hipMemcpy(c->d_tap_off, off.data(), off.size() * sizeof(unsigned long long), hipMemcpyHostToDevice) != hipSuccess)
            return fail(TMAC_HIP_E_RUNTIME, "tap offsets: allocation failed");
    }
    c->tap = dev_buffer;
    return TMAC_HIP_OK;
}

extern "C" int32_t tmac_hip_chain_set_stamps(tmac_hip_chain* c, unsigned long long* dev_buffer) {
    if (!c) return fail(TMAC_HIP_E_ARG, "null chain");
#ifndef TMAC_STREAM_STAMPS
    if (c->stream && dev_buffer) return fail(TMAC_HIP_E_NOMATCH, "stamps of a stream-mode chain exist in -DTMAC_STREAM_STAMPS builds only (layout: StreamArgs::stamps)");
#endif
    if (!c->stream && dev_buffer && !TMAC_CHAIN_STAMPS)
        return fail(TMAC_HIP_E_NOMATCH, "stamps of k_decode_chain exist in -DTMAC_CHAIN_STAMPS=1 builds of the library only (tools/build_variant.sh)");
    c->stamps = dev_buffer;
    return TMAC_HIP_OK;
}

extern "C" int32_t tmac_hip_chain_threads(void) { return CHAIN_FT; }

extern "C" int32_t tmac_hip_chain_is_stream(const tmac_hip_chain* c) { return c && c->stream ? (c->qw ? 2 : 1) : 0; }
```

tmac_amd/csrc/tmac_stream.hip:

```cpp
#include <hip/hip_runtime.h>
#include <hip/hip_fp16.h>
#include <stdint.h>

#include "tmac_chain_core.h"

#ifndef TMAC_STREAM_QW_TU
#define TMAC_STREAM_QW_TU 0
#endif
#ifndef TMAC_STREAM_G2_TU
#define TMAC_STREAM_G2_TU 0
#endif

namespace tmac {

#if !TMAC_STREAM_QW_TU && !TMAC_STREAM_G2_TU
__global__ __launch_bounds__(256) void k_lut_images(const ChainOp* __restrict__ ops) {
    const ChainOp& d = ops[blockIdx.y];
    const int K = d.K, P = K / 8, nst = d.nst;
    if ((int)blockIdx.x >= nst) return;
    const int p = blockIdx.x * 256 + threadIdx.x;
    uint4* tab = reinterpret_cast<uint4*>(const_cast<void*>(d.img));
    float* l_sc = reinterpret_cast<float*>(tab + IMG2_STEP * nst);
    uint4* tslot = tab + img2_index(p >> 2, p & 3);
#if TMAC_IMG2_SC
    float* scslot = l_sc + 4 * (p >> 4) + ((p >> 3) & 1);
#else
    float* scslot = l_sc + (p >> 3);
#endif
    if (p >= P) {
        *tslot = make_uint4(0u, 0u, 0u, 0u);
        if ((p & 7) == 0) { scslot[0] = 0.f; scslot[TMAC_IMG2_SC ? 2 : 32 * nst] = 0.f; }
        return;
    }
    float x[8];
    if (d.in_gran & 2) {
        const float4* src = reinterpret_cast<const float4*>(d.in) + 2 * (size_t)p;
        const float4 a0 = src[0], a1 = src[1];
        x[0] = a0.x; x[1] = a0.y; x[2] = a0.z; x[3] = a0.w; x[4] = a1.x; x[5] = a1.y; x[6] = a1.z; x[7] = a1.w;
    } else {
        const uint4 v = reinterpret_cast<const uint4*>(d.in)[p];
        const uint32_t r[4] = {v.x, v.y, v.z, v.w};
#pragma unroll
        for (int i = 0; i < 4; ++i) {
            const __half2 hh = *reinterpret_cast<const __half2*>(&r[i]);
            x[2 * i] = __low2float(hh); x[2 * i + 1] = __high2float(hh);
        }
    }
    const float s0 = __fadd_rn(__fadd_rn(fabsf(x[0]), fabsf(x[1])), __fadd_rn(fabsf(x[2]), fabsf(x[3])));
    const float s1 = __fadd_rn(__fadd_rn(fabsf(x[4]), fabsf(x[5])), __fadd_rn(fabsf(x[6]), fabsf(x[7])));
    const float mx = q_half_allmax(fmaxf(s0, s1));
    const float scales = div127(mx);
    const float t_scales = (scales != 0.0f) ? rcp_exact(scales) : 0.0f;
    uint32_t lo0, hi0, lo1, hi1;
    float La, Lb;
    q_table8<true>(x[0], x[1], x[2], x[3], t_scales, lo0, hi0, La);
    q_table8<true>(x[4], x[5], x[6], x[7], t_scales, lo1, hi1, Lb);
    *tslot = make_uint4(lo0, hi0, lo1, hi1);
    float va = -La, vb = -Lb;
    va = __fadd_rn(va, qdpp_f<0x4E>(va));
    vb = __fadd_rn(vb, qdpp_f<0x4E>(vb));
    va = __fadd_rn(va, qdpp_f<0xB1>(va));
    vb = __fadd_rn(vb, qdpp_f<0xB1>(vb));
    const float v = __fadd_rn(va, vb);
    const float c1 = qdpp_f<0x104>(v);
    if ((p & 7) == 0) {
        scslot[0] = __fmul_rn(0.5f, scales);
        scslot[TMAC_IMG2_SC ? 2 : 32 * nst] = __fmul_rn(0.5f, __fadd_rn(__fadd_rn(0.0f, v), c1));
    }
}

template <bool SCF16>
__global__ __launch_bounds__(256) void k_lut_images_us(const ChainOp* __restrict__ ops) {
    __shared__ float s_cs[768];
    __shared__ float s_mx[4];
    const ChainOp& d = ops[blockIdx.x];
    const int K = d.K, P = K / 8, nu = d.nu, nst = d.nst;
    const int tid = threadIdx.x, w = tid >> 6, lane = tid & 63;
    uint4* tab = reinterpret_cast<uint4*>(const_cast<void*>(d.img));
    float* l_us = reinterpret_cast<float*>(tab + IMG2_STEP * nst);
    auto load8 = [&](int p, float (&x)[8]) __attribute__((always_inline)) {
        if (d.in_gran & 2) {
            const float4* src = reinterpret_cast<const float4*>(d.in) + 2 * (size_t)p;
            const float4 a0 = src[0], a1 = src[1];
            x[0] = a0.x; x[1] = a0.y; x[2] = a0.z; x[3] = a0.w; x[4] = a1.x; x[5] = a1.y; x[6] = a1.z; x[7] = a1.w;
        } else {
            const uint4 v = reinterpret_cast<const uint4*>(d.in)[p];
            const uint32_t r[4] = {v.x, v.y, v.z, v.w};
#pragma unroll
            for (int i = 0; i < 4; ++i) {
                const __half2 hh = *reinterpret_cast<const __half2*>(&r[i]);
                x[2 * i] = __low2float(hh); x[2 * i + 1] = __high2float(hh);
            }
        }
    };
    float mx = 0.f;
    for (int p = tid; p < P; p += 256) {
        float x[8];
        load8(p, x);
        mx = fmaxf(mx, __fadd_rn(__fadd_rn(fabsf(x[0]), fabsf(x[1])), __fadd_rn(fabsf(x[2]), fabsf(x[3]))));
        mx = fmaxf(mx, __fadd_rn(__fadd_rn(fabsf(x[4]), fabsf(x[5])), __fadd_rn(fabsf(x[6]), fabsf(x[7]))));
        float va = -__fadd_rn(__fadd_rn(__fadd_rn(x[0], x[1]), x[2]), x[3]);
        float vb = -__fadd_rn(__fadd_rn(__fadd_rn(x[4], x[5]), x[6]), x[7]);
        va = __fadd_rn(va, qdpp_f<0x4E>(va));
        vb = __fadd_rn(vb, qdpp_f<0x4E>(vb));
        va = __fadd_rn(va, qdpp_f<0xB1>(va));
        vb = __fadd_rn(vb, qdpp_f<0xB1>(vb));
        if ((p & 3) == 0) s_cs[p >> 2] = __fadd_rn(va, vb);
    }
    mx = q_row_allmax(mx);
    mx = q_xor_max_f(mx);
    if (lane == 0) s_mx[w] = mx;
    __syncthreads();
    mx = fmaxf(fmaxf(s_mx[0], s_mx[1]), fmaxf(s_mx[2], s_mx[3]));
    const float gscale = div127(mx);
    const float gtinv = (gscale != 0.0f) ? rcp_exact(gscale) : 0.0f;
    for (int p = tid; p < P; p += 256) {
        float x[8];
        load8(p, x);
        uint32_t lo0, hi0, lo1, hi1;
        float La, Lb;
        q_table8<true>(x[0], x[1], x[2], x[3], gtinv, lo0, hi0, La);
        q_table8<true>(x[4], x[5], x[6], x[7], gtinv, lo1, hi1, Lb);
        tab[img2_index(p >> 2, p & 3)] = make_uint4(lo0, hi0, lo1, hi1);
    }
    for (int j4 = 0; j4 < 4; ++j4)
        for (int u = nu + tid; u < nst * 64; u += 256) tab[img2_index(u, j4)] = make_uint4(0u, 0u, 0u, 0u);
    if (tid == 0) {
        float biases = 0.0f;
        for (int c = 0; c < nu; ++c) biases = __fadd_rn(biases, s_cs[c]);
        l_us[0] = gscale;
        l_us[1] = biases;
    }
    if (tid >= 64 && tid < 64 + 4 * CHAIN_US_MAX_GROUPS) {
        const int mi = (tid - 64) / CHAIN_US_MAX_GROUPS, g = (tid - 64) % CHAIN_US_MAX_GROUPS;
        if (mi < d.nmat && g < d.m_groups)
            l_us[16 + mi * CHAIN_US_MAX_GROUPS + g] = SCF16 ? __half2float(reinterpret_cast<const __half*>(d.m[mi].SC)[g]) : reinterpret_cast<const float*>(d.m[mi].SC)[g];
    }
}

hipError_t launch_lut_images(const ChainOp* d_ops, int nops, int max_nst, int sm, bool sc_f16, hipStream_t st) {
    if (nops < 1 || max_nst < 1) return hipErrorInvalidValue;
    if (sm == 2 && sc_f16) hipLaunchKernelGGL(k_lut_images_us<true>, dim3(nops), dim3(256), 0, st, d_ops);
    else if (sm == 2) hipLaunchKernelGGL(k_lut_images_us<false>, dim3(nops), dim3(256), 0, st, d_ops);
    else hipLaunchKernelGGL(k_lut_images, dim3(max_nst, nops), dim3(256), 0, st, d_ops);
    return hipGetLastError();
}
#endif

#ifndef TMAC_STREAM_KO
#define TMAC_STREAM_KO 0
#endif
#define TMAC_STREAM_ATTR __attribute__((amdgpu_num_sgpr(82)))
template <int BITS, bool ZP, bool SCF16, int RING, int MINW, int SM, bool TAP, bool QW, bool G2 = false>
__global__ __launch_bounds__(STREAM_FT, MINW) TMAC_STREAM_ATTR void k_gemv_stream(StreamArgs a) {
    extern __shared__ __attribute__((aligned(16))) uint4 lds[];
    constexpr int NWV = STREAM_NLW;
    constexpr int RPW = QW ? 16 : 4;
    const int tid = threadIdx.x, w = __builtin_amdgcn_readfirstlane(tid >> 6), lane = tid & 63;
    const int nsplit = a.nsplit, part = (int)blockIdx.x % nsplit, bx = (int)blockIdx.x / nsplit;
    const int cls = __builtin_amdgcn_readfirstlane(bx * a.ncls / ((int)gridDim.x / nsplit));
    const int* my_roles = a.roles + (size_t)cls * a.vmax * STREAM_ROLE_INTS;
    const int nops = max((a.nvis[cls] - part + nsplit - 1) / nsplit, 0);
    if (nops == 0) return;
    float* l_red = reinterpret_cast<float*>(lds + 2 * (size_t)a.buf_u4);
    uint4* l_ops = lds + 2 * (size_t)a.buf_u4 + (2 * NWV * RPW * CHAIN_RED * sizeof(float)) / 16;
    {
        constexpr int U = (int)(sizeof(ChainOp) / 16);
        const uint4* gsrc = reinterpret_cast<const uint4*>(a.ops);
        for (int idx = tid; idx < nops * U; idx += STREAM_FT) {
            const int jl = idx / U, r = idx - jl * U;
            l_ops[idx] = gsrc[my_roles[(size_t)(jl * nsplit + part) * STREAM_ROLE_INTS + SR_OP] * U + r];
        }
        __syncthreads();
    }
    const cop_ptr ops = reinterpret_cast<cop_ptr>(l_ops);
    auto wg_iters = [&](cop_ptr d) __attribute__((always_inline)) {
        const int qper = uni(d->q_per), qex = uni(d->q_extra), ipi = uni(d->ipi), iinv = uni(d->ipi_inv), bl = bx - uni(d->wg_lo);
        const int cnt = qper + (bl < qex ? 1 : 0);
        return ((cnt + ipi - 1) * iinv) >> 16;
    };

    if (w == NWV) {
        typedef __attribute__((address_space(3))) void* lds_vp;
        const uint32_t lds0 = (uint32_t)(uintptr_t)(__attribute__((address_space(3))) uint4*)lds;
        auto load_image = [&](int j) __attribute__((always_inline)) {
            const cop_ptr d = ops + j;
            const int n16 = uni(d->img_u4);
            const __amdgpu_buffer_rsrc_t rs = __builtin_amdgcn_make_buffer_rsrc(const_cast<void*>(uni(d->img)), (short)0, n16 * 16, 0x00020000);
            const uint32_t base = lds0 + (uint32_t)(j & 1) * (uint32_t)a.buf_u4 * 16u;
            for (int o = 0; o < n16; o += 64)
                __builtin_amdgcn_raw_ptr_buffer_load_lds(rs, (lds_vp)(uintptr_t)(base + (uint32_t)o * 16u), 16, (o + lane) * 16, 0, 0, 0);
        };
        int s_par = 0;
        auto combine = [&](int j, int t, int par) __attribute__((always_inline)) {
            const cop_ptr d = ops + j;
            const int qper = uni(d->q_per), qex = uni(d->q_extra), ipi = uni(d->ipi), wpq = uni(d->wpq), bl = bx - uni(d->wg_lo);
            const int q_lo = bl * qper + min(bl, qex), cnt = qper + (bl < qex ? 1 : 0);
            constexpr int SPP = 64 / RPW;
            for (int pass = 0; pass * SPP < ipi; ++pass) {
            const int p_qs = pass * SPP + (int)((unsigned)lane / RPW), p_row = lane & (RPW - 1);
            const int p_gql = q_lo + t * ipi + p_qs;
            if (p_qs < ipi && p_gql < q_lo + cnt) {
                const int e0 = uni(d->q_end[0]), e1 = uni(d->q_end[1]), e2 = uni(d->q_end[2]);
                const int p_mi = (p_gql >= e0 ? 1 : 0) + (p_gql >= e1 ? 1 : 0) + (p_gql >= e2 ? 1 : 0);
                const int p_lq = p_gql - (p_gql >= e2 ? e2 : (p_gql >= e1 ? e1 : (p_gql >= e0 ? e0 : 0)));
                const unsigned long long p_c = reinterpret_cast<unsigned long long>(d->m[p_mi].C);
                const float* red = l_red + par * (NWV * RPW * CHAIN_RED);
                float v;
                if (SM == 2) {
                    int32_t cb[BITS];
#pragma unroll
                    for (int pl = 0; pl < BITS; ++pl) cb[pl] = 0;
                    const int32_t* redi = reinterpret_cast<const int32_t*>(red);
                    for (int ww = 0; ww < wpq; ++ww)
#pragma unroll
                        for (int pl = 0; pl < BITS; ++pl) cb[pl] += redi[((p_qs * wpq + ww) * RPW + p_row) * CHAIN_RED + pl];
                    if constexpr (TAP) {
                        if (a.tap) {
                            const int opi = my_roles[(size_t)(j * nsplit + part) * STREAM_ROLE_INTS + SR_OP];
#pragma unroll
                            for (int pl = 0; pl < BITS; ++pl) a.tap[a.tap_off[opi] + (size_t)(RPW * p_gql + p_row) * BITS + pl] = cb[pl];
                        }
                    }
                    float acc = 0.f;
#pragma unroll
                    for (int pl = 0; pl < BITS; ++pl) {
                        const float tp = __fmul_rn((float)cb[pl], q_alpha(pl));
                        acc = (pl == 0) ? tp : __fadd_rn(acc, tp);
                    }
                    const float* l_us = reinterpret_cast<const float*>(lds + (size_t)(j & 1) * a.buf_u4 + IMG2_STEP * (size_t)uni(d->nst));
                    const float vv = __fadd_rn(__fmul_rn(acc, l_us[0]), __fmul_rn(l_us[1], 0.5f));
                    const int mg = uni(d->m_groups);
                    const int g = mg == 1 ? 0 : (RPW * p_lq + p_row) / (d->m[p_mi].Mw / mg);
                    v = __fmul_rn(vv, l_us[16 + p_mi * CHAIN_US_MAX_GROUPS + g]);
                } else {
                v = red[((p_qs * wpq) * RPW + p_row) * CHAIN_RED];
                for (int ww = 1; ww < wpq; ++ww) v = __fadd_rn(v, red[((p_qs * wpq + ww) * RPW + p_row) * CHAIN_RED]);
                }
                asm volatile("" : "+v"(v));
                const size_t oi = (size_t)(RPW * p_lq + p_row);
                if (a.out_f16) c_store_b16(p_c + 2 * oi, (uint32_t)__half_as_ushort(__float2half_rn(v)));
                else c_store_b32(p_c + 4 * oi, __float_as_uint(v));
            }
            }
        };
        load_image(0);
        int prev_nit = 0;
        for (int j = 0; j < nops; ++j) {
            asm volatile("s_waitcnt vmcnt(0)" ::: "memory");
            c_lds_barrier();
            if (!(TMAC_STREAM_KO & 1) && j > 0 && prev_nit > 0) combine(j - 1, prev_nit - 1, s_par ^ 1);
            if (!(TMAC_STREAM_KO & 4) && j + 1 < nops) load_image(j + 1);
            const int nit = wg_iters(ops + j);
            if (!(TMAC_STREAM_KO & 2))
                for (int t = 0; t < nit; ++t) {
                    c_lds_barrier();
                    if (!(TMAC_STREAM_KO & 1) && t + 1 < nit) combine(j, t, s_par);
                    s_par ^= 1;
                }
            prev_nit = nit;
        }
        if (!(TMAC_STREAM_KO & 1) && prev_nit > 0) combine(nops - 1, prev_nit - 1, s_par ^ 1);
        return;
    }

    CSel<BITS> sel;
    c_selectors<BITS, SM>(sel, lane);
    uint32_t k3 = 0x03020100u;
    asm volatile("" : "+v"(k3));
    uint32_t lane16 = QW ? (uint32_t)(lane & 15) * 16u : (uint32_t)lane * 16u;
    asm volatile("" : "+v"(lane16));
    uint32_t lk4 = QW ? 8u * (uint32_t)(lane >> 4)
                      : 4u * (uint32_t)(2 * (lane & 12) + 2 * (lane >> 4));
    asm volatile("" : "+v"(lk4));
    const int wl = NWV - 1 - w;

    typedef int sr16 __attribute__((ext_vector_type(16)));
    typedef int sr4 __attribute__((ext_vector_type(4)));
    auto load_role = [&](int jl, sr16& rc, sr4& rw) __attribute__((always_inline)) {
        const int* rp = my_roles + (size_t)(jl * nsplit + part) * STREAM_ROLE_INTS;
        const int* rpw = rp + SR_COMMON + SRW_INTS * wl;
        asm volatile("s_load_dwordx16 %0, %2, 0x0\n\ts_load_dwordx4 %1, %3, 0x0\n\ts_waitcnt lgkmcnt(0)" : "=&s"(rc), "=&s"(rw) : "s"(rp), "s"(rpw) : "memory");
    };
    auto items_of = [&](const sr16& rc, const sr4& rw) __attribute__((always_inline)) {
        const int nq = bx - rc[SR_WLO] < rc[SR_QEXTRA] ? (int)((unsigned)rw[SRW_NQ] >> 16) : (rw[SRW_NQ] & 0xffff);
        return nq * rw[SRW_NSTEPS];
    };

    CFrag<BITS, G2> ring[RING];
    const __amdgpu_buffer_rsrc_t null_rs = __builtin_amdgcn_make_buffer_rsrc(static_cast<uint4*>(nullptr), (short)0, 0, 0x00020000);
    const TMAC_GLOBAL char* ops_g = as_global(reinterpret_cast<const char*>(a.ops));
    const uint32_t dummy_boff = (uint32_t)(lane & 3) * (uint32_t)((ZP ? 2 : 1) * (SCF16 ? 2 : 4));
    uint32_t v_sc0 = dummy_boff;
    bool i_rag = false;
    uint32_t v_wq = lane16, v_scq = dummy_boff;
    int i_op = -1, i_left = 0, i_st = 0, i_h = 0, i_wpq = 1, i_nst = 1, i_nsg1 = 0, i_gsh = 0, i_nu = 0, i_gq = 0, i_ipi = 1, i_n64 = 1;
    int q_lo = 0, q_hi = 0, q_woff = 0;
    bool q_stale = true;
    cop_ptr i_d = ops;
    __amdgpu_buffer_rsrc_t q_rs = null_rs;
    const TMAC_GLOBAL char* q_sc = ops_g;
    const TMAC_GLOBAL char* q_scm = ops_g;
    int q_scstride = 0;
    const uint32_t c0 = QW ? (uint32_t)(4 * (lane >> 4)) : (uint32_t)(4 * (lane & 12) + 4 * (lane >> 4));
    uint32_t c0g = c0;
    int i_sc2 = 0;
    constexpr int SC_SHIFT = (ZP ? 1 : 0) + (SCF16 ? 3 : 4);
    auto refill = [&](CFrag<BITS, G2>& f) __attribute__((always_inline)) {
        while (i_left == 0 && i_op < nops) {
            ++i_op;
            if (i_op < nops) {
                i_d = ops + i_op;
                sr16 rc; sr4 rw;
                load_role(i_op, rc, rw);
                i_left = items_of(rc, rw);
                i_st = rw[SRW_H]; i_h = rw[SRW_H]; i_wpq = rc[SR_WPQ]; i_nst = rc[SR_NST]; i_ipi = rc[SR_IPI];
                const int bl = bx - rc[SR_WLO];
                i_gq = bl * rc[SR_QPER] + min(bl, rc[SR_QEXTRA]) + rw[SRW_QS];
                i_nsg1 = rc[SR_NSG] - 1; i_gsh = rc[SR_GSH]; i_nu = rc[SR_NU];
                q_scstride = rc[SR_NSG] << SC_SHIFT;
                c0g = c0 >> i_gsh;
                if constexpr (G2) i_sc2 = i_gsh < 2 ? 1 << SC_SHIFT : 0;
                if constexpr (QW) {
                    i_n64 = (rc[SR_TSTRIDE] - 1) >> 6;
                    v_wq = (uint32_t)(lane >> 4) * (uint32_t)(i_n64 * (BITS * 1024)) + lane16;
                    v_scq = (uint32_t)((lane >> 2) & 3) * (uint32_t)q_scstride + dummy_boff;
                    v_sc0 = (c0g << SC_SHIFT) + v_scq;
                    i_rag = (i_nu & 15) != 0;
                } else {
                    v_sc0 = (c0g << SC_SHIFT) | dummy_boff;
                    i_rag = (i_nu & 63) != 0;
                }
                q_hi = 0; q_stale = true;
            }
        }
        const bool real = i_left > 0;
        if (real && q_stale) {
            if (i_gq >= q_hi) {
                const int e0 = uni(i_d->q_end[0]), e1 = uni(i_d->q_end[1]), e2 = uni(i_d->q_end[2]);
                const int mi = (i_gq >= e0 ? 1 : 0) + (i_gq >= e1 ? 1 : 0) + (i_gq >= e2 ? 1 : 0);
                q_lo = i_gq >= e2 ? e2 : (i_gq >= e1 ? e1 : (i_gq >= e0 ? e0 : 0));
                q_hi = i_gq >= e2 ? 0x7fffffff : (i_gq >= e1 ? e2 : (i_gq >= e0 ? e1 : e0));
                q_rs = __builtin_amdgcn_make_buffer_rsrc(const_cast<uint4*>(uni(i_d->m[mi].W)), (short)0, 0x7fffffff, 0x00020000);
                q_scm = as_global(uni(reinterpret_cast<const char*>(i_d->m[mi].SC)));
            }
            const int lq = QW ? 4 * (i_gq - q_lo) : i_gq - q_lo;
            q_sc = q_scm + (size_t)lq * (size_t)q_scstride;
            q_woff = lq * (QW ? i_n64 : i_nst) * (BITS * 1024);
            q_stale = false;
        }
        CItemOps io;
        if (real) {
            io.rs = q_rs;
            const int ub = QW ? i_st << 4 : i_st << 6;
            if (i_rag && i_st == i_nst - 1) {
                const uint32_t sg = min((uint32_t)(ub >> i_gsh) + c0g, (uint32_t)i_nsg1);
                io.sc = q_sc;
                io.boff = QW ? (sg << SC_SHIFT) + v_scq : ((sg << SC_SHIFT) | dummy_boff);
                if constexpr (G2) {
                    const uint32_t sg2 = min((uint32_t)(ub >> i_gsh) + c0g + (uint32_t)(i_sc2 >> SC_SHIFT), (uint32_t)i_nsg1);
                    io.boff2 = QW ? (sg2 << SC_SHIFT) + v_scq : ((sg2 << SC_SHIFT) | dummy_boff);
                }
                io.l16 = QW ? v_wq : ((lane < i_nu - ub) ? lane16 : 0u);
            } else {
                io.sc = q_sc + ((size_t)(ub >> i_gsh) << SC_SHIFT);
                io.boff = v_sc0;
                if constexpr (G2) io.boff2 = v_sc0 + (uint32_t)i_sc2;
                io.l16 = QW ? v_wq : lane16;
            }
            io.soff = QW ? q_woff + (i_st >> 2) * (BITS * 1024) + (i_st & 3) * 256 : q_woff + i_st * (BITS * 1024);
        } else { io.rs = null_rs; io.soff = 0; io.sc = ops_g; io.boff = dummy_boff; io.l16 = 0u; if constexpr (G2) io.boff2 = dummy_boff; }
        c_issue_static<BITS, ZP, SCF16, SM, G2>(f, io);
        if (real) {
            --i_left;
            i_st += i_wpq;
            if (i_st >= i_nst) { i_st = i_h; i_gq += i_ipi; q_stale = true; }
        }
    };
#pragma unroll
    for (int k = 0; k < RING; ++k) refill(ring[k]);

    int c_op = -1, c_left = 0, c_it = 0, c_st = 0, parity = 0, my_iter = 0;
    int tstride = 1, nst = 1, wpq = 1, h = 0;
    int t_gq0 = 0, t_ipi = 1, t_G = 0;
    int32_t* t_base = nullptr;
    uint4* tab = lds;
    float* l_ls = reinterpret_cast<float*>(lds);
    float* l_lb = l_ls;
    float cacc = 0.f;
    int32_t iacc[BITS];
#pragma unroll
    for (int pl = 0; pl < BITS; ++pl) iacc[pl] = 0;

#ifdef TMAC_STREAM_STAMPS
    uint32_t* t_lds = reinterpret_cast<uint32_t*>(l_ops) + (size_t)nops * (sizeof(ChainOp) / 4) + (size_t)w * 8;
    if (lane < 8) t_lds[lane] = 0;
    uint32_t t_prev = (uint32_t)__builtin_readcyclecounter();
#if TMAC_STREAM_STAMPS >= 2
    if (lane == 0) t_lds[7] = 0u - t_prev;
#else
    if (lane == 0) { t_lds[6] = t_prev; t_lds[7] = (uint32_t)(__builtin_readcyclecounter() >> 32); }
#endif
#if TMAC_STREAM_STAMPS >= 2
#define TMAC_ST(i) do { const uint32_t t_now = (uint32_t)__builtin_readcyclecounter(); if (lane == 0) (void)__hip_atomic_fetch_add(&t_lds[i], t_now - t_prev, __ATOMIC_RELAXED, __HIP_MEMORY_SCOPE_WORKGROUP); t_prev = t_now; } while (0)
#else
#define TMAC_ST(i) do { } while (0)
#endif
#else
#define TMAC_ST(i) do { } while (0)
#endif
    auto finish = [&](bool have, float acc_in) __attribute__((always_inline)) {
        if (TMAC_STREAM_KO & 2) { ++c_it; return; }
        float* red = l_red + parity * (NWV * RPW * CHAIN_RED);
        if (SM == 2) {
            int32_t* redi = reinterpret_cast<int32_t*>(red);
#pragma unroll
            for (int pl = 0; pl < BITS; ++pl) {
                uint32_t v = have ? (uint32_t)iacc[pl] : 0u;
                if constexpr (!QW) {
                    v += qdpp_u<0x124>(v);
                    v += qdpp_u<0x128>(v);
                }
                v = q_xor_add_u(v);
                if (lane < RPW) redi[(wl * RPW + lane) * CHAIN_RED + pl] = (int32_t)v;
                iacc[pl] = 0;
            }
        } else {
        float acc = 0.f;
        if (have) {
            acc = acc_in;
            if constexpr (!QW) {
                acc = __fadd_rn(acc, qdpp_f<0x124>(acc));
                acc = __fadd_rn(acc, qdpp_f<0x128>(acc));
            }
            acc = q_xor_add_f(acc);
        }
        if (lane < RPW) red[(wl * RPW + lane) * CHAIN_RED] = acc;
        }
        TMAC_ST(2);
        c_lds_barrier();
        TMAC_ST(3);
        parity ^= 1;
        ++c_it;
    };
    bool done = false;
    auto advance = [&]() __attribute__((always_inline)) {
        for (;;) {
            if (c_op >= 0) while (c_it < my_iter) finish(false, 0.f);
            ++c_op;
            if (c_op >= nops) { done = true; return; }
            sr16 rc; sr4 rw;
            load_role(c_op, rc, rw);
            my_iter = bx - rc[SR_WLO] < rc[SR_QEXTRA] ? rc[SR_IT_HI] : rc[SR_IT_LO];
            tstride = rc[SR_TSTRIDE]; nst = rc[SR_NST]; wpq = rc[SR_WPQ]; h = rw[SRW_H];
            tab = lds + (size_t)(c_op & 1) * a.buf_u4;
            l_ls = reinterpret_cast<float*>(tab + IMG2_STEP * ((tstride - 1) >> 6));
            l_lb = TMAC_IMG2_SC ? l_ls : l_ls + ((tstride - 1) >> 1);
            c_left = items_of(rc, rw); c_it = 0; c_st = h;
            if constexpr (TAP) {
                const int bl = bx - rc[SR_WLO];
                t_gq0 = bl * rc[SR_QPER] + min(bl, rc[SR_QEXTRA]) + rw[SRW_QS]; t_ipi = rc[SR_IPI]; t_G = rc[SR_NU] >> 1;
                t_base = a.tap ? a.tap + a.tap_off[rc[SR_OP]] : nullptr;
            }
            TMAC_ST(4);
            c_lds_barrier();
            TMAC_ST(5);
            if (c_left > 0) return;
        }
    };

    advance();
    while (!done) {
#pragma unroll
        for (int k = 0; k < RING; ++k) {
            if (!done) {
#if defined(TMAC_STREAM_STAMPS) && TMAC_STREAM_STAMPS >= 2
                {
                    constexpr int L = BITS + (G2 ? 2 : 1) * (SCF16 || !ZP ? 1 : 2);
                    asm volatile("s_waitcnt vmcnt(%0)" :: "n"((RING - 1) * L) : "memory");
                    TMAC_ST(0);
                    if (lane == 0) (void)__hip_atomic_fetch_add(&t_lds[6], 1u, __ATOMIC_RELAXED, __HIP_MEMORY_SCOPE_WORKGROUP);
                }
#endif
                if (TMAC_STREAM_KO & 8) cacc += __uint_as_float(ring[k].wq[0].x ^ ring[k].wq[BITS - 1].w ^ ring[k].s0); else
                c_compute<BITS, ZP, SCF16, SM, TAP, true, G2>(ring[k], tab, tstride, l_ls, l_lb, QW ? c_st * 16 : c_st * 64, lane16, lk4, sel, k3, cacc, iacc,
                                                          (TAP && t_base) ? t_base + (size_t)(RPW * (t_gq0 + c_it * t_ipi) + (lane & (RPW - 1))) * t_G : nullptr, t_G,
                                                          QW ? (c_st >> 2) * (16 * IMG2_STEP) + (c_st & 3) * 256 : c_st * (16 * IMG2_STEP));
                asm volatile("" : "+v"(cacc));
            }
            refill(ring[k]);
            TMAC_ST(1);
            if (!done) {
                --c_left;
                c_st += wpq;
                if (c_st >= nst) {
                    finish(true, cacc);
                    cacc = 0.f;
                    c_st = h;
                }
                if (c_left == 0) advance();
                TMAC_ST(4);
            }
        }
    }
#ifdef TMAC_STREAM_STAMPS
    if (a.stamps && lane == 0) {
        const unsigned long long t_last = __builtin_readcyclecounter();
        unsigned long long* o = a.stamps + ((size_t)blockIdx.x * NWV + w) * 8;
#if TMAC_STREAM_STAMPS >= 2
        for (int i = 0; i < 7; ++i) o[i] = t_lds[i];
        uint32_t hw_id2;
        asm volatile("s_getreg_b32 %0, hwreg(HW_REG_HW_ID)" : "=s"(hw_id2));
        o[7] = (unsigned long long)(uint32_t)(t_lds[7] + (uint32_t)t_last) | ((unsigned long long)hw_id2 << 32);
#else
        const unsigned long long t_first = ((unsigned long long)t_lds[7] << 32) | t_lds[6];
        o[4] = t_last - t_first;
        uint32_t hw_id, xcc_id;
        asm volatile("s_getreg_b32 %0, hwreg(HW_REG_HW_ID)" : "=s"(hw_id));
        asm volatile("s_getreg_b32 %0, hwreg(HW_REG_XCC_ID)" : "=s"(xcc_id));
        o[5] = t_first; o[6] = t_last; o[7] = ((unsigned long long)xcc_id << 32) | hw_id;
#endif
    }
#endif
#undef TMAC_ST

}

template <int BITS, bool QWF, bool G2F>
static hipError_t stream_launch_b(const StreamArgs& a, bool zp, bool sc_f16, int sm, int grid, size_t lds_bytes, hipStream_t st) {
    constexpr int R2 = G2F ? ((BITS <= 2) ? 2 : 1) : ((BITS <= 3) ? 2 : 1);
    constexpr int R1 = (BITS <= 2) ? 4 : 2;
#define TMAC_SL2(Z, H, R, MW, S) do { \
        auto* kern = a.tap ? &k_gemv_stream<BITS, Z, H, R1, 4, S, true, QWF, G2F> : &k_gemv_stream<BITS, Z, H, R, MW, S, false, QWF, G2F>; \
        if (lds_bytes > 64 * 1024) { \
            hipError_t e = hipFuncSetAttribute(reinterpret_cast<const void*>(kern), hipFuncAttributeMaxDynamicSharedMemorySize, (int)lds_bytes); \
            if (e != hipSuccess) return e; \
        } \
        hipLaunchKernelGGL(kern, dim3(grid * a.nsplit), dim3(STREAM_FT), lds_bytes, st, a); \
        return hipGetLastError(); } while (0)
#define TMAC_SL(Z, H, S) do { if constexpr (!(G2F && BITS == 4)) { if (a.nsplit >= 2) TMAC_SL2(Z, H, R2, 8, S); } TMAC_SL2(Z, H, R1, 4, S); } while (0)
    if constexpr (!G2F) {
        if (sm == 2) { if (sc_f16) TMAC_SL(false, true, 2); else TMAC_SL(false, false, 2); }
    } else if (sm != 0) return hipErrorInvalidValue;
    if (zp) { if (sc_f16) TMAC_SL(true, true, 0); else TMAC_SL(true, false, 0); }
    if (sc_f16) TMAC_SL(false, true, 0);
    TMAC_SL(false, false, 0);
#undef TMAC_SL
#undef TMAC_SL2
}

#define TMAC_STREAM_BITS_SWITCH(QWF, G2F) \
    switch (bits) { \
        case 1: return stream_launch_b<1, QWF, G2F>(a, zp, sc_f16, sm, grid, lds_bytes, st); \
        case 2: return stream_launch_b<2, QWF, G2F>(a, zp, sc_f16, sm, grid, lds_bytes, st); \
        case 3: return stream_launch_b<3, QWF, G2F>(a, zp, sc_f16, sm, grid, lds_bytes, st); \
        case 4: return stream_launch_b<4, QWF, G2F>(a, zp, sc_f16, sm, grid, lds_bytes, st); \
        default: return hipErrorInvalidValue; \
    }
#if TMAC_STREAM_QW_TU && TMAC_STREAM_G2_TU
hipError_t launch_gemv_stream_qw_g2(const StreamArgs& a, int bits, bool zp, bool sc_f16, int sm, int grid, size_t lds_bytes, hipStream_t st) {
    TMAC_STREAM_BITS_SWITCH(true, true)
}
#elif TMAC_STREAM_G2_TU
hipError_t launch_gemv_stream_g2(const StreamArgs& a, int bits, bool zp, bool sc_f16, int sm, int grid, size_t lds_bytes, hipStream_t st) {
    TMAC_STREAM_BITS_SWITCH(false, true)
}
#elif TMAC_STREAM_QW_TU
hipError_t launch_gemv_stream_qw(const StreamArgs& a, int bits, bool zp, bool sc_f16, int sm, int grid, size_t lds_bytes, hipStream_t st) {
    TMAC_STREAM_BITS_SWITCH(true, false)
}
#else
hipError_t launch_gemv_stream_qw(const StreamArgs& a, int bits, bool zp, bool sc_f16, int sm, int grid, size_t lds_bytes, hipStream_t st);
hipError_t launch_gemv_stream_g2(const StreamArgs& a, int bits, bool zp, bool sc_f16, int sm, int grid, size_t lds_bytes, hipStream_t st);
hipError_t launch_gemv_stream_qw_g2(const StreamArgs& a, int bits, bool zp, bool sc_f16, int sm, int grid, size_t lds_bytes, hipStream_t st);
hipError_t launch_gemv_stream(const StreamArgs& a, int bits, bool zp, bool sc_f16, int sm, bool qw, bool g2, int grid, size_t lds_bytes, hipStream_t st) {
    if (a.nops < 1 || grid < 1 || a.nsplit < 1 || a.nsplit > 4 || (sm != 0 && sm != 2) || (g2 && sm != 0)) return hipErrorInvalidValue;
    if (g2) return qw ? launch_gemv_stream_qw_g2(a, bits, zp, sc_f16, sm, grid, lds_bytes, st) : launch_gemv_stream_g2(a, bits, zp, sc_f16, sm, grid, lds_bytes, st);
    if (qw) return launch_gemv_stream_qw(a, bits, zp, sc_f16, sm, grid, lds_bytes, st);
    TMAC_STREAM_BITS_SWITCH(false, false)
}
#endif
#undef TMAC_STREAM_BITS_SWITCH

}
```

Baseline: 6597.

## Precompute per-slot entry blocks and LUT block list; hoist LDS attribute setup

The stream kernel now reads per-class visit counts from packed kernel arguments instead of a device array. It loads each workgroup's op descriptors from a precomputed contiguous entry block laid out per (class, split, slot). The LUT image kernel launches one workgroup per real (op, step) block from a flat descriptor list, so it no longer spawns a max_nst x nops grid with early-exit blocks. The per-launch hipFuncSetAttribute call moves to commit time behind a mutex-guarded per-device cache, cutting host overhead on every launch, and timing stamps are extended. The cost is extra device memory for the entry block, plus a host-side failure when a class makes more than 0xffff visits or there are more than 16 classes.

```diff
diff --git a/include/tmac_hip.h b/include/tmac_hip.h
--- a/include/tmac_hip.h
+++ b/include/tmac_hip.h
@@ -124,6 +124,8 @@
 int32_t tmac_hip_debug_chain_config(int force_waves_per_quad, unsigned spin_limit);
 int32_t tmac_hip_debug_chain_grid(int workgroups);
 int32_t tmac_hip_debug_stream_schedule(const double* items, int n, int grid, int ncls, int target, int lpt, int32_t* out_lo, int32_t* out_w, double* out_load);
+int32_t tmac_hip_debug_stream_entry(const double* items, int n, int grid, int ncls, int target, int lpt, int nsplit, int32_t* out_nvis, int32_t* out_visits,
+                                    int vcap, int32_t* out_counts, int32_t* out_vper, int32_t* out_slots, int slot_cap);
 
 #define TMAC_HIP_COMM_ID_BYTES 128
 typedef struct tmac_hip_comm tmac_hip_comm;
diff --git a/tmac_amd/binding.py b/tmac_amd/binding.py
--- a/tmac_amd/binding.py
+++ b/tmac_amd/binding.py
@@ -138,6 +138,8 @@
         "tmac_hip_chain_connect": ([vp, vp, C.c_int], i32),
         "tmac_hip_debug_chain_grid": ([C.c_int], i32),
         "tmac_hip_debug_stream_schedule": ([C.POINTER(C.c_double), C.c_int, C.c_int, C.c_int, C.c_int, C.c_int, C.POINTER(C.c_int32), C.POINTER(C.c_int32), C.POINTER(C.c_double)], i32),
+        "tmac_hip_debug_stream_entry": ([C.POINTER(C.c_double), C.c_int, C.c_int, C.c_int, C.c_int, C.c_int, C.c_int, C.POINTER(C.c_int32), C.POINTER(C.c_int32), C.c_int,
+                                        C.POINTER(C.c_int32), C.POINTER(C.c_int32), C.POINTER(C.c_int32), C.c_int], i32),
         "tmac_hip_debug_chain_config": ([C.c_int, C.c_uint], i32),
         "tmac_hip_debug_quad_config": ([C.c_int, C.c_int], i32),
         "tmac_hip_selftest": ([vp, vp, C.c_int], i32),
@@ -147,7 +149,7 @@
         "preprocessor_int8": ([C.c_int] * 4 + [vp] * 4, i32),
     }
     optional = {"tmac_hip_chain_is_stream", "tmac_hip_chain_xform", "tmac_hip_qgemm_fused_xf_dev", "tmac_hip_qgemm_fused_xf_rows_dev", "tmac_hip_debug_xf_rows", "tmac_hip_debug_xf_rows_plan", "tmac_hip_debug_fused_plan", "tmac_hip_debug_route_stats", "tmac_hip_comm_init_ipc", "tmac_hip_comm_export", "tmac_hip_comm_connect", "tmac_hip_comm_status",
-                "tmac_hip_debug_rows_kernel", "tmac_hip_debug_rows_stats", "tmac_hip_debug_rows_plan", "tmac_hip_debug_rows_comb_sums"} if os.environ.get("TMAC_HIP_LIB") else set()
+                "tmac_hip_debug_stream_entry", "tmac_hip_debug_rows_kernel", "tmac_hip_debug_rows_stats", "tmac_hip_debug_rows_plan", "tmac_hip_debug_rows_comb_sums"} if os.environ.get("TMAC_HIP_LIB") else set()
     for name, (argt, rest) in sigs.items():
         try:
             fn = getattr(L, name)
diff --git a/tmac_amd/csrc/tmac_chain.h b/tmac_amd/csrc/tmac_chain.h
--- a/tmac_amd/csrc/tmac_chain.h
+++ b/tmac_amd/csrc/tmac_chain.h
@@ -131,7 +131,9 @@
     int nsplit;
     int ncls;
     int vmax;
-    const int* nvis;
+    unsigned long long nvis_pk[4];
+    const ChainOp* entry;
+    int vper;
     const int* roles;
     int32_t* tap;
     const unsigned long long* tap_off;
@@ -149,7 +151,16 @@
 #endif
     return b;
 }
-hipError_t launch_lut_images(const ChainOp* d_ops, int nops, int max_nst, int sm, bool sc_f16, hipStream_t st);
-hipError_t launch_gemv_stream(const StreamArgs& a, int bits, bool zp, bool sc_f16, int sm, bool qw, bool g2, int grid, size_t lds_bytes, hipStream_t st);
+struct LutBlock {
+    const void* in;
+    void* img;
+    int K, nst;
+    int in_gran;
+    int step;
+};
+static_assert(sizeof(LutBlock) == 32, "LutBlock is read with one scalar load");
+hipError_t launch_lut_images(const ChainOp* d_ops, int nops, const LutBlock* blocks, int nblocks, int sm, bool sc_f16, hipStream_t st);
+hipError_t launch_gemv_stream(const StreamArgs& a, int bits, bool zp, bool sc_f16, int sm, bool qw, bool g2, int grid, size_t lds_bytes, hipStream_t st,
+                              bool prepare = false);
 
 }
diff --git a/tmac_amd/csrc/tmac_chain_host.cpp b/tmac_amd/csrc/tmac_chain_host.cpp
--- a/tmac_amd/csrc/tmac_chain_host.cpp
+++ b/tmac_amd/csrc/tmac_chain_host.cpp
@@ -177,6 +177,46 @@
                 out_load[k] += it[i] / wg;
             }
         }
+    return TMAC_HIP_OK;
+}
+
+static bool stream_entry_layout(const std::vector<std::vector<int>>& visits, int nsplit, std::vector<int>& slot_op, int& vper, unsigned long long (&nvis_pk)[4]) {
+    const int ncls = (int)visits.size();
+    size_t vmax = 1;
+    for (const std::vector<int>& v : visits) vmax = std::max(vmax, v.size());
+    vper = (int)((vmax + nsplit - 1) / nsplit);
+    slot_op.assign((size_t)ncls * nsplit * vper, -1);
+    for (int k = 0; k < 4; ++k) nvis_pk[k] = 0;
+    if (ncls > 16) return false;
+    for (int c = 0; c < ncls; ++c) {
+        if (visits[c].size() > 0xffffu) return false;
+        nvis_pk[c >> 2] |= (unsigned long long)visits[c].size() << (16 * (c & 3));
+        for (size_t v = 0; v < visits[c].size(); ++v)
+            slot_op[((size_t)c * nsplit + v % nsplit) * vper + v / nsplit] = visits[c][v];
+    }
+    return true;
+}
+extern "C" int32_t tmac_hip_debug_stream_entry(const double* items, int n, int grid, int ncls, int target, int lpt, int nsplit, int32_t* out_nvis, int32_t* out_visits,
+                                               int vcap, int32_t* out_counts, int32_t* out_vper, int32_t* out_slots, int slot_cap) {
+    if (!items || n < 1 || grid < 1 || ncls < 1 || ncls > 16 || (ncls & (ncls - 1)) || ncls > grid || nsplit < 1 || nsplit > 4 || !out_nvis || !out_visits || !out_counts ||
+        !out_vper || !out_slots || vcap < 1)
+        return fail(TMAC_HIP_E_ARG, "bad entry-block query");
+    std::vector<double> it(items, items + n);
+    std::vector<int> lo, w, slots;
+    std::vector<std::vector<int>> vis;
+    stream_schedule(it, grid, ncls, target, lpt != 0, lo, w, vis);
+    int vper = 0;
+    unsigned long long pk[4];
+    if (!stream_entry_layout(vis, nsplit, slots, vper, pk)) return fail(TMAC_HIP_E_NOMATCH, "a class' visit count does not fit the kernel's argument");
+    if ((int)slots.size() > slot_cap) return fail(TMAC_HIP_E_ARG, "the entry block has %zu slots, room for %d", slots.size(), slot_cap);
+    for (int c = 0; c < ncls; ++c) {
+        if ((int)vis[c].size() > vcap) return fail(TMAC_HIP_E_ARG, "class %d makes %zu visits, room for %d", c, vis[c].size(), vcap);
+        out_nvis[c] = (int32_t)vis[c].size();
+        out_counts[c] = (int32_t)((pk[c >> 2] >> (16 * (c & 3))) & 0xffffu);
+        for (int v = 0; v < vcap; ++v) out_visits[(size_t)c * vcap + v] = v < (int)vis[c].size() ? vis[c][v] : -1;
+    }
+    *out_vper = vper;
+    for (size_t k = 0; k < slots.size(); ++k) out_slots[k] = slots[k];
     return TMAC_HIP_OK;
 }
 
@@ -500,8 +540,10 @@
     std::vector<ChainOp> ops;
     std::vector<size_t> img_off;
     std::vector<int32_t> roles;
+    std::vector<int> slot_op;
+    unsigned long long nvis_pk[4] = {0, 0, 0, 0};
     size_t img_bytes = 0, lds_bytes = 0;
-    int buf_u4 = 0, max_nst = 0, ncls = 1, vmax = 1, nsplit = 1;
+    int buf_u4 = 0, ncls = 1, vmax = 1, vper = 1, nsplit = 1;
     bool qw = true;
 };
 static std::optional<StreamPlan> plan_stream(std::vector<ChainOp> ops, int bits, bool g2, int grid, const BuildKnobs& kn) {
@@ -515,7 +557,6 @@
         p.img_off[i] = p.img_bytes;
         p.img_bytes += (size_t)o.img_u4 * 16;
         if (o.img_u4 > p.buf_u4) p.buf_u4 = o.img_u4;
-        if (o.nst > p.max_nst) p.max_nst = o.nst;
         o.in_gran &= 2;
     }
     const int nwv = STREAM_NLW;
@@ -559,9 +600,9 @@
         if (p.nsplit == ns - 1 && vmax >= ns && ns * (ldsn + 1024) <= 160 * 1024) { p.nsplit = ns; p.lds_bytes = ldsn; }
     }
     if (p.lds_bytes > 160 * 1024) return std::nullopt;
-    p.roles.assign((size_t)STREAM_ROLE_INTS * ncls * vmax + ncls, 0);
+    if (!stream_entry_layout(visits, p.nsplit, p.slot_op, p.vper, p.nvis_pk)) return std::nullopt;
+    p.roles.assign((size_t)STREAM_ROLE_INTS * ncls * vmax, 0);
     for (int k = 0; k < ncls; ++k) {
-        p.roles[(size_t)STREAM_ROLE_INTS * ncls * vmax + k] = (int32_t)visits[k].size();
         for (size_t v = 0; v < visits[k].size(); ++v) {
             const int i = visits[k][v];
             const ChainOp& o = p.ops[i];
@@ -586,16 +627,38 @@
 }
 
 static int32_t commit_stream(tmac_hip_chain& c, StreamPlan& p) {
-    const size_t role_bytes = p.roles.size() * sizeof(int32_t);
-    if (hipMalloc(&c.images, p.img_bytes + role_bytes) != hipSuccess || hipMemset(c.images, 0, p.img_bytes) != hipSuccess ||
-        hipMemcpy(static_cast<char*>(c.images) + p.img_bytes, p.roles.data(), role_bytes, hipMemcpyHostToDevice) != hipSuccess)
-        return fail(TMAC_HIP_E_RUNTIME, "LUT image allocation failed (%zu bytes)", p.img_bytes + role_bytes);
-    c.roles = reinterpret_cast<const int*>(static_cast<char*>(c.images) + p.img_bytes);
-    c.nvis = c.roles + (size_t)STREAM_ROLE_INTS * p.ncls * p.vmax;
-    c.ncls = p.ncls; c.vmax = p.vmax; c.qw = p.qw; c.nsplit = p.nsplit; c.max_nst = p.max_nst;
+    const size_t role_bytes = (p.roles.size() * sizeof(int32_t) + 255) & ~(size_t)255;
+    const size_t entry_bytes = p.slot_op.size() * sizeof(ChainOp);
+    std::vector<ChainOp> entry(p.slot_op.size());
+    std::vector<LutBlock> blocks;
+    size_t nblk = 0;
+    if (c.sm != 2) for (const ChainOp& o : p.ops) nblk += (size_t)o.nst;
+    if (hipMalloc(&c.images, p.img_bytes + role_bytes + entry_bytes + nblk * sizeof(LutBlock)) != hipSuccess || hipMemset(c.images, 0, p.img_bytes) != hipSuccess)
+        return fail(TMAC_HIP_E_RUNTIME, "LUT image allocation failed (%zu bytes)", p.img_bytes + role_bytes + entry_bytes + nblk * sizeof(LutBlock));
+    char* const dev = static_cast<char*>(c.images);
     c.ops = std::move(p.ops);
-    for (size_t i = 0; i < c.ops.size(); ++i) c.ops[i].img = static_cast<const char*>(c.images) + p.img_off[i];
+    for (size_t i = 0; i < c.ops.size(); ++i) c.ops[i].img = dev + p.img_off[i];
+    memset(entry.data(), 0, entry_bytes);
+    for (size_t k = 0; k < entry.size(); ++k) if (p.slot_op[k] >= 0) entry[k] = c.ops[p.slot_op[k]];
+    if (c.sm != 2)
+        for (const ChainOp& o : c.ops)
+            for (int st = 0; st < o.nst; ++st) blocks.push_back(LutBlock{o.in, const_cast<void*>(o.img), o.K, o.nst, o.in_gran, st});
+    if (hipMemcpy(dev + p.img_bytes, p.roles.data(), p.roles.size() * sizeof(int32_t), hipMemcpyHostToDevice) != hipSuccess ||
+        hipMemcpy(dev + p.img_bytes + role_bytes, entry.data(), entry_bytes, hipMemcpyHostToDevice) != hipSuccess ||
+        (nblk && hipMemcpy(dev + p.img_bytes + role_bytes + entry_bytes, blocks.data(), nblk * sizeof(LutBlock), hipMemcpyHostToDevice) != hipSuccess))
+        return fail(TMAC_HIP_E_RUNTIME, "upload of the stream's role records and entry block failed");
+    c.roles = reinterpret_cast<const int*>(dev + p.img_bytes);
+    c.entry = reinterpret_cast<const ChainOp*>(dev + p.img_bytes + role_bytes);
+    c.lut_blocks = nblk ? reinterpret_cast<const LutBlock*>(dev + p.img_bytes + role_bytes + entry_bytes) : nullptr;
+    c.n_lut_blocks = (int)nblk;
+    memcpy(c.nvis_pk, p.nvis_pk, sizeof(c.nvis_pk));
+    c.ncls = p.ncls; c.vmax = p.vmax; c.vper = p.vper; c.qw = p.qw; c.nsplit = p.nsplit;
     c.stream = true; c.buf_u4 = p.buf_u4; c.lds_bytes = p.lds_bytes; c.xforms = 0;
+    StreamArgs sa;
+    memset(&sa, 0, sizeof(sa));
+    sa.nops = (int)c.ops.size(); sa.nsplit = c.nsplit;
+    const hipError_t e = launch_gemv_stream(sa, c.bits, c.zp != 0, c.sc_f16 != 0, c.sm, c.qw, c.g2 != 0, c.grid, c.lds_bytes, nullptr, true);
+    if (e != hipSuccess) return fail(TMAC_HIP_E_RUNTIME, "stream kernel with %zu bytes of LDS: %s", c.lds_bytes, hipGetErrorString(e));
     return TMAC_HIP_OK;
 }
 static int32_t commit(tmac_hip_chain& c, const ChainLayout& lay) {
diff --git a/tmac_amd/csrc/tmac_chain_host.h b/tmac_amd/csrc/tmac_chain_host.h
--- a/tmac_amd/csrc/tmac_chain_host.h
+++ b/tmac_amd/csrc/tmac_chain_host.h
@@ -27,9 +27,12 @@
     bool launched = false;
     bool stream = false;
     void* images = nullptr;
-    int max_nst = 0;
     const int* roles = nullptr;
-    const int* nvis = nullptr;
+    unsigned long long nvis_pk[4] = {0, 0, 0, 0};
+    const tmac::ChainOp* entry = nullptr;
+    int vper = 0;
+    const tmac::LutBlock* lut_blocks = nullptr;
+    int n_lut_blocks = 0;
     int ncls = 1, vmax = 0;
     bool qw = false;
     int nsplit = 1;
diff --git a/tmac_amd/csrc/tmac_chain_launch.cpp b/tmac_amd/csrc/tmac_chain_launch.cpp
--- a/tmac_amd/csrc/tmac_chain_launch.cpp
+++ b/tmac_amd/csrc/tmac_chain_launch.cpp
@@ -14,12 +14,12 @@
     }
     if (!c->connected) return fail(TMAC_HIP_E_ARG, "a row-sharded chain must be connected to its peers first (tmac_hip_chain_export / tmac_hip_chain_connect)");
     if (c->stream) {
-        hipError_t e = launch_lut_images(c->d_ops, (int)c->ops.size(), c->max_nst, c->sm, c->sc_f16 != 0, st);
+        hipError_t e = launch_lut_images(c->d_ops, (int)c->ops.size(), c->lut_blocks, c->n_lut_blocks, c->sm, c->sc_f16 != 0, st);
         if (e != hipSuccess) return fail(TMAC_HIP_E_RUNTIME, "LUT image launch: %s", hipGetErrorString(e));
         StreamArgs sa;
         memset(&sa, 0, sizeof(sa));
         sa.ops = c->d_ops; sa.nops = (int)c->ops.size(); sa.out_f16 = c->out_f16; sa.buf_u4 = c->buf_u4; sa.nsplit = c->nsplit; sa.roles = c->roles; sa.stamps = c->stamps;
-        sa.ncls = c->ncls; sa.vmax = c->vmax; sa.nvis = c->nvis; sa.tap = c->tap; sa.tap_off = c->d_tap_off;
+        sa.ncls = c->ncls; sa.vmax = c->vmax; sa.entry = c->entry; sa.vper = c->vper; memcpy(sa.nvis_pk, c->nvis_pk, sizeof(sa.nvis_pk)); sa.tap = c->tap; sa.tap_off = c->d_tap_off;
         e = launch_gemv_stream(sa, c->bits, c->zp != 0, c->sc_f16 != 0, c->sm, c->qw, c->g2 != 0, c->grid, c->lds_bytes, st);
         if (e != hipSuccess) return fail(TMAC_HIP_E_RUNTIME, "stream launch: %s", hipGetErrorString(e));
         c->last_stream = st; c->launched = true;
diff --git a/tmac_amd/csrc/tmac_stream.hip b/tmac_amd/csrc/tmac_stream.hip
--- a/tmac_amd/csrc/tmac_stream.hip
+++ b/tmac_amd/csrc/tmac_stream.hip
@@ -1,6 +1,7 @@
 #include <hip/hip_runtime.h>
 #include <hip/hip_fp16.h>
 #include <stdint.h>
+#include <mutex>
 
 #include "tmac_chain_core.h"
 
@@ -14,12 +15,11 @@
 namespace tmac {
 
 #if !TMAC_STREAM_QW_TU && !TMAC_STREAM_G2_TU
-__global__ __launch_bounds__(256) void k_lut_images(const ChainOp* __restrict__ ops) {
-    const ChainOp& d = ops[blockIdx.y];
+__global__ __launch_bounds__(256) void k_lut_images(const LutBlock* __restrict__ blocks) {
+    const LutBlock d = blocks[blockIdx.x];
     const int K = d.K, P = K / 8, nst = d.nst;
-    if ((int)blockIdx.x >= nst) return;
-    const int p = blockIdx.x * 256 + threadIdx.x;
-    uint4* tab = reinterpret_cast<uint4*>(const_cast<void*>(d.img));
+    const int p = d.step * 256 + threadIdx.x;
+    uint4* tab = reinterpret_cast<uint4*>(d.img);
     float* l_sc = reinterpret_cast<float*>(tab + IMG2_STEP * nst);
     uint4* tslot = tab + img2_index(p >> 2, p & 3);
 #if TMAC_IMG2_SC
@@ -138,11 +138,11 @@
     }
 }
 
-hipError_t launch_lut_images(const ChainOp* d_ops, int nops, int max_nst, int sm, bool sc_f16, hipStream_t st) {
-    if (nops < 1 || max_nst < 1) return hipErrorInvalidValue;
+hipError_t launch_lut_images(const ChainOp* d_ops, int nops, const LutBlock* blocks, int nblocks, int sm, bool sc_f16, hipStream_t st) {
+    if (nops < 1 || (sm != 2 && (nblocks < 1 || !blocks))) return hipErrorInvalidValue;
     if (sm == 2 && sc_f16) hipLaunchKernelGGL(k_lut_images_us<true>, dim3(nops), dim3(256), 0, st, d_ops);
     else if (sm == 2) hipLaunchKernelGGL(k_lut_images_us<false>, dim3(nops), dim3(256), 0, st, d_ops);
-    else hipLaunchKernelGGL(k_lut_images, dim3(max_nst, nops), dim3(256), 0, st, d_ops);
+    else hipLaunchKernelGGL(k_lut_images, dim3(nblocks), dim3(256), 0, st, blocks);
     return hipGetLastError();
 }
 #endif
@@ -157,23 +157,42 @@
     constexpr int NWV = STREAM_NLW;
     constexpr int RPW = QW ? 16 : 4;
     const int tid = threadIdx.x, w = __builtin_amdgcn_readfirstlane(tid >> 6), lane = tid & 63;
+#if defined(TMAC_STREAM_STAMPS) && TMAC_STREAM_STAMPS == 1
+    const unsigned long long t_entry = __builtin_amdgcn_s_memrealtime();
+#endif
     const int nsplit = a.nsplit, part = (int)blockIdx.x % nsplit, bx = (int)blockIdx.x / nsplit;
     const int cls = __builtin_amdgcn_readfirstlane(bx * a.ncls / ((int)gridDim.x / nsplit));
     const int* my_roles = a.roles + (size_t)cls * a.vmax * STREAM_ROLE_INTS;
-    const int nops = max((a.nvis[cls] - part + nsplit - 1) / nsplit, 0);
+    const unsigned long long nv_pk = cls < 8 ? (cls < 4 ? a.nvis_pk[0] : a.nvis_pk[1]) : (cls < 12 ? a.nvis_pk[2] : a.nvis_pk[3]);
+    const int nops = max(((int)((nv_pk >> (16 * (cls & 3))) & 0xffffu) - part + nsplit - 1) / nsplit, 0);
     if (nops == 0) return;
     float* l_red = reinterpret_cast<float*>(lds + 2 * (size_t)a.buf_u4);
     uint4* l_ops = lds + 2 * (size_t)a.buf_u4 + (2 * NWV * RPW * CHAIN_RED * sizeof(float)) / 16;
-    {
+    const TMAC_GLOBAL ChainOp* g_ent = as_global(a.entry) + (size_t)((cls * nsplit + part) * a.vper);
+    typedef __attribute__((address_space(3))) void* lds_vp;
+    const uint32_t lds0 = (uint32_t)(uintptr_t)(__attribute__((address_space(3))) uint4*)lds;
+    auto issue_image = [&](const void* img, int n16, int buf) __attribute__((always_inline)) {
+        const __amdgpu_buffer_rsrc_t rs = __builtin_amdgcn_make_buffer_rsrc(const_cast<void*>(img), (short)0, n16 * 16, 0x00020000);
+        const uint32_t base = lds0 + (uint32_t)buf * (uint32_t)a.buf_u4 * 16u;
+        for (int o = 0; o < n16; o += 64)
+            __builtin_amdgcn_raw_ptr_buffer_load_lds(rs, (lds_vp)(uintptr_t)(base + (uint32_t)o * 16u), 16, (o + lane) * 16, 0, 0, 0);
+    };
+    if (w == NWV) {
+        issue_image(uni(g_ent->img), uni(g_ent->img_u4), 0);
+    } else {
         constexpr int U = (int)(sizeof(ChainOp) / 16);
-        const uint4* gsrc = reinterpret_cast<const uint4*>(a.ops);
-        for (int idx = tid; idx < nops * U; idx += STREAM_FT) {
-            const int jl = idx / U, r = idx - jl * U;
-            l_ops[idx] = gsrc[my_roles[(size_t)(jl * nsplit + part) * STREAM_ROLE_INTS + SR_OP] * U + r];
-        }
-        __syncthreads();
-    }
+        typedef uint32_t u32x4 __attribute__((ext_vector_type(4)));
+        const TMAC_GLOBAL u32x4* gsrc = reinterpret_cast<const TMAC_GLOBAL u32x4*>(g_ent);
+        for (int idx = tid; idx < nops * U; idx += NWV * 64) reinterpret_cast<u32x4*>(l_ops)[idx] = gsrc[idx];
+    }
+    c_lds_barrier();
     const cop_ptr ops = reinterpret_cast<cop_ptr>(l_ops);
+#if defined(TMAC_STREAM_STAMPS) && TMAC_STREAM_STAMPS == 1
+    if (lane == 0) {
+        uint32_t* t0 = reinterpret_cast<uint32_t*>(l_ops) + (size_t)nops * (sizeof(ChainOp) / 4) + (size_t)w * 8;
+        t0[0] = (uint32_t)t_entry; t0[1] = (uint32_t)(t_entry >> 32);
+    }
+#endif
     auto wg_iters = [&](cop_ptr d) __attribute__((always_inline)) {
         const int qper = uni(d->q_per), qex = uni(d->q_extra), ipi = uni(d->ipi), iinv = uni(d->ipi_inv), bl = bx - uni(d->wg_lo);
         const int cnt = qper + (bl < qex ? 1 : 0);
@@ -181,15 +200,9 @@
     };
 
     if (w == NWV) {
-        typedef __attribute__((address_space(3))) void* lds_vp;
-        const uint32_t lds0 = (uint32_t)(uintptr_t)(__attribute__((address_space(3))) uint4*)lds;
         auto load_image = [&](int j) __attribute__((always_inline)) {
             const cop_ptr d = ops + j;
-            const int n16 = uni(d->img_u4);
-            const __amdgpu_buffer_rsrc_t rs = __builtin_amdgcn_make_buffer_rsrc(const_cast<void*>(uni(d->img)), (short)0, n16 * 16, 0x00020000);
-            const uint32_t base = lds0 + (uint32_t)(j & 1) * (uint32_t)a.buf_u4 * 16u;
-            for (int o = 0; o < n16; o += 64)
-                __builtin_amdgcn_raw_ptr_buffer_load_lds(rs, (lds_vp)(uintptr_t)(base + (uint32_t)o * 16u), 16, (o + lane) * 16, 0, 0, 0);
+            issue_image(uni(d->img), uni(d->img_u4), j & 1);
         };
         int s_par = 0;
         auto combine = [&](int j, int t, int par) __attribute__((always_inline)) {
@@ -244,7 +257,6 @@
             }
             }
         };
-        load_image(0);
         int prev_nit = 0;
         for (int j = 0; j < nops; ++j) {
             asm volatile("s_waitcnt vmcnt(0)" ::: "memory");
@@ -261,6 +273,12 @@
             prev_nit = nit;
         }
         if (!(TMAC_STREAM_KO & 1) && prev_nit > 0) combine(nops - 1, prev_nit - 1, s_par ^ 1);
+#if defined(TMAC_STREAM_STAMPS) && TMAC_STREAM_STAMPS == 1
+        if (a.stamps && lane == 0) {
+            asm volatile("s_waitcnt vmcnt(0)" ::: "memory");
+            a.stamps[((size_t)blockIdx.x * NWV + 0) * 8 + 3] = __builtin_amdgcn_s_memrealtime();
+        }
+#endif
         return;
     }
 
@@ -394,12 +412,18 @@
 
 #ifdef TMAC_STREAM_STAMPS
     uint32_t* t_lds = reinterpret_cast<uint32_t*>(l_ops) + (size_t)nops * (sizeof(ChainOp) / 4) + (size_t)w * 8;
+#if TMAC_STREAM_STAMPS >= 2
     if (lane < 8) t_lds[lane] = 0;
+#endif
     uint32_t t_prev = (uint32_t)__builtin_readcyclecounter();
 #if TMAC_STREAM_STAMPS >= 2
     if (lane == 0) t_lds[7] = 0u - t_prev;
 #else
-    if (lane == 0) { t_lds[6] = t_prev; t_lds[7] = (uint32_t)(__builtin_readcyclecounter() >> 32); }
+    if (lane == 0) {
+        const unsigned long long t_iss = __builtin_amdgcn_s_memrealtime();
+        t_lds[2] = (uint32_t)t_iss; t_lds[3] = (uint32_t)(t_iss >> 32);
+        t_lds[6] = t_prev; t_lds[7] = (uint32_t)(__builtin_readcyclecounter() >> 32);
+    }
 #endif
 #if TMAC_STREAM_STAMPS >= 2
 #define TMAC_ST(i) do { const uint32_t t_now = (uint32_t)__builtin_readcyclecounter(); if (lane == 0) (void)__hip_atomic_fetch_add(&t_lds[i], t_now - t_prev, __ATOMIC_RELAXED, __HIP_MEMORY_SCOPE_WORKGROUP); t_prev = t_now; } while (0)
@@ -470,6 +494,12 @@
     };
 
     advance();
+#if defined(TMAC_STREAM_STAMPS) && TMAC_STREAM_STAMPS == 1
+    if (lane == 0) {
+        const unsigned long long t_a0 = __builtin_amdgcn_s_memrealtime();
+        t_lds[4] = (uint32_t)t_a0; t_lds[5] = (uint32_t)(t_a0 >> 32);
+    }
+#endif
     while (!done) {
 #pragma unroll
         for (int k = 0; k < RING; ++k) {
@@ -514,6 +544,10 @@
         o[7] = (unsigned long long)(uint32_t)(t_lds[7] + (uint32_t)t_last) | ((unsigned long long)hw_id2 << 32);
 #else
         const unsigned long long t_first = ((unsigned long long)t_lds[7] << 32) | t_lds[6];
+        o[0] = ((unsigned long long)t_lds[1] << 32) | t_lds[0];
+        o[1] = ((unsigned long long)t_lds[3] << 32) | t_lds[2];
+        o[2] = ((unsigned long long)t_lds[5] << 32) | t_lds[4];
+        if (w != 0) o[3] = __builtin_amdgcn_s_memrealtime();
         o[4] = t_last - t_first;
         uint32_t hw_id, xcc_id;
         asm volatile("s_getreg_b32 %0, hwreg(HW_REG_HW_ID)" : "=s"(hw_id));
@@ -526,17 +560,30 @@
 
 }
 
+constexpr int STREAM_MAX_DEVICES = 64;
 template <int BITS, bool QWF, bool G2F>
-static hipError_t stream_launch_b(const StreamArgs& a, bool zp, bool sc_f16, int sm, int grid, size_t lds_bytes, hipStream_t st) {
+static hipError_t stream_launch_b(const StreamArgs& a, bool zp, bool sc_f16, int sm, int grid, size_t lds_bytes, hipStream_t st, bool prepare) {
     constexpr int R2 = G2F ? ((BITS <= 2) ? 2 : 1) : ((BITS <= 3) ? 2 : 1);
     constexpr int R1 = (BITS <= 2) ? 4 : 2;
 #define TMAC_SL2(Z, H, R, MW, S) do { \
-        auto* kern = a.tap ? &k_gemv_stream<BITS, Z, H, R1, 4, S, true, QWF, G2F> : &k_gemv_stream<BITS, Z, H, R, MW, S, false, QWF, G2F>; \
-        if (lds_bytes > 64 * 1024) { \
-            hipError_t e = hipFuncSetAttribute(reinterpret_cast<const void*>(kern), hipFuncAttributeMaxDynamicSharedMemorySize, (int)lds_bytes); \
-            if (e != hipSuccess) return e; \
+        auto* kern_t = &k_gemv_stream<BITS, Z, H, R1, 4, S, true, QWF, G2F>; \
+        auto* kern_p = &k_gemv_stream<BITS, Z, H, R, MW, S, false, QWF, G2F>; \
+        if (prepare) {       \
+             \
+            static size_t raised[STREAM_MAX_DEVICES]; \
+            static std::mutex mu; \
+            int dev = 0; \
+            hipError_t e = hipGetDevice(&dev); \
+            if (e != hipSuccess || lds_bytes <= 64 * 1024) return e; \
+            if (dev < 0 || dev >= STREAM_MAX_DEVICES) return hipErrorInvalidDevice; \
+            std::lock_guard<std::mutex> lock(mu); \
+            if (lds_bytes <= raised[dev]) return hipSuccess; \
+            e = hipFuncSetAttribute(reinterpret_cast<const void*>(kern_p), hipFuncAttributeMaxDynamicSharedMemorySize, (int)lds_bytes); \
+            if (e == hipSuccess) e = hipFuncSetAttribute(reinterpret_cast<const void*>(kern_t), hipFuncAttributeMaxDynamicSharedMemorySize, (int)lds_bytes); \
+            if (e == hipSuccess) raised[dev] = lds_bytes; \
+            return e; \
         } \
-        hipLaunchKernelGGL(kern, dim3(grid * a.nsplit), dim3(STREAM_FT), lds_bytes, st, a); \
+        hipLaunchKernelGGL(a.tap ? kern_t : kern_p, dim3(grid * a.nsplit), dim3(STREAM_FT), lds_bytes, st, a); \
         return hipGetLastError(); } while (0)
 #define TMAC_SL(Z, H, S) do { if constexpr (!(G2F && BITS == 4)) { if (a.nsplit >= 2) TMAC_SL2(Z, H, R2, 8, S); } TMAC_SL2(Z, H, R1, 4, S); } while (0)
     if constexpr (!G2F) {
@@ -551,32 +598,32 @@
 
 #define TMAC_STREAM_BITS_SWITCH(QWF, G2F) \
     switch (bits) { \
-        case 1: return stream_launch_b<1, QWF, G2F>(a, zp, sc_f16, sm, grid, lds_bytes, st); \
-        case 2: return stream_launch_b<2, QWF, G2F>(a, zp, sc_f16, sm, grid, lds_bytes, st); \
-        case 3: return stream_launch_b<3, QWF, G2F>(a, zp, sc_f16, sm, grid, lds_bytes, st); \
-        case 4: return stream_launch_b<4, QWF, G2F>(a, zp, sc_f16, sm, grid, lds_bytes, st); \
+        case 1: return stream_launch_b<1, QWF, G2F>(a, zp, sc_f16, sm, grid, lds_bytes, st, prepare); \
+        case 2: return stream_launch_b<2, QWF, G2F>(a, zp, sc_f16, sm, grid, lds_bytes, st, prepare); \
+        case 3: return stream_launch_b<3, QWF, G2F>(a, zp, sc_f16, sm, grid, lds_bytes, st, prepare); \
+        case 4: return stream_launch_b<4, QWF, G2F>(a, zp, sc_f16, sm, grid, lds_bytes, st, prepare); \
         default: return hipErrorInvalidValue; \
     }
 #if TMAC_STREAM_QW_TU && TMAC_STREAM_G2_TU
-hipError_t launch_gemv_stream_qw_g2(const StreamArgs& a, int bits, bool zp, bool sc_f16, int sm, int grid, size_t lds_bytes, hipStream_t st) {
+hipError_t launch_gemv_stream_qw_g2(const StreamArgs& a, int bits, bool zp, bool sc_f16, int sm, int grid, size_t lds_bytes, hipStream_t st, bool prepare) {
     TMAC_STREAM_BITS_SWITCH(true, true)
 }
 #elif TMAC_STREAM_G2_TU
-hipError_t launch_gemv_stream_g2(const StreamArgs& a, int bits, bool zp, bool sc_f16, int sm, int grid, size_t lds_bytes, hipStream_t st) {
+hipError_t launch_gemv_stream_g2(const StreamArgs& a, int bits, bool zp, bool sc_f16, int sm, int grid, size_t lds_bytes, hipStream_t st, bool prepare) {
     TMAC_STREAM_BITS_SWITCH(false, true)
 }
 #elif TMAC_STREAM_QW_TU
-hipError_t launch_gemv_stream_qw(const StreamArgs& a, int bits, bool zp, bool sc_f16, int sm, int grid, size_t lds_bytes, hipStream_t st) {
+hipError_t launch_gemv_stream_qw(const StreamArgs& a, int bits, bool zp, bool sc_f16, int sm, int grid, size_t lds_bytes, hipStream_t st, bool prepare) {
     TMAC_STREAM_BITS_SWITCH(true, false)
 }
 #else
-hipError_t launch_gemv_stream_qw(const StreamArgs& a, int bits, bool zp, bool sc_f16, int sm, int grid, size_t lds_bytes, hipStream_t st);
-hipError_t launch_gemv_stream_g2(const StreamArgs& a, int bits, bool zp, bool sc_f16, int sm, int grid, size_t lds_bytes, hipStream_t st);
-hipError_t launch_gemv_stream_qw_g2(const StreamArgs& a, int bits, bool zp, bool sc_f16, int sm, int grid, size_t lds_bytes, hipStream_t st);
-hipError_t launch_gemv_stream(const StreamArgs& a, int bits, bool zp, bool sc_f16, int sm, bool qw, bool g2, int grid, size_t lds_bytes, hipStream_t st) {
+hipError_t launch_gemv_stream_qw(const StreamArgs& a, int bits, bool zp, bool sc_f16, int sm, int grid, size_t lds_bytes, hipStream_t st, bool prepare);
+hipError_t launch_gemv_stream_g2(const StreamArgs& a, int bits, bool zp, bool sc_f16, int sm, int grid, size_t lds_bytes, hipStream_t st, bool prepare);
+hipError_t launch_gemv_stream_qw_g2(const StreamArgs& a, int bits, bool zp, bool sc_f16, int sm, int grid, size_t lds_bytes, hipStream_t st, bool prepare);
+hipError_t launch_gemv_stream(const StreamArgs& a, int bits, bool zp, bool sc_f16, int sm, bool qw, bool g2, int grid, size_t lds_bytes, hipStream_t st, bool prepare) {
     if (a.nops < 1 || grid < 1 || a.nsplit < 1 || a.nsplit > 4 || (sm != 0 && sm != 2) || (g2 && sm != 0)) return hipErrorInvalidValue;
-    if (g2) return qw ? launch_gemv_stream_qw_g2(a, bits, zp, sc_f16, sm, grid, lds_bytes, st) : launch_gemv_stream_g2(a, bits, zp, sc_f16, sm, grid, lds_bytes, st);
-    if (qw) return launch_gemv_stream_qw(a, bits, zp, sc_f16, sm, grid, lds_bytes, st);
+    if (g2) return qw ? launch_gemv_stream_qw_g2(a, bits, zp, sc_f16, sm, grid, lds_bytes, st, prepare) : launch_gemv_stream_g2(a, bits, zp, sc_f16, sm, grid, lds_bytes, st, prepare);
+    if (qw) return launch_gemv_stream_qw(a, bits, zp, sc_f16, sm, grid, lds_bytes, st, prepare);
     TMAC_STREAM_BITS_SWITCH(false, false)
 }
 #endif
```

Result: no change. 6596 (-0.0%).
